# slowkow/scde

Hardware: NVIDIA B200
Metric: genes/sec scde.expression.difference (100 boot) (higher is better)
Workload: dtype f64 + s8 fixed point (2^-29, exact int32 sums)

## Files before the change

### scde_b200/csrc/api.cu

```cuda
#include "../../include/scde_b200.h"
#include "common.cuh"
#include "hostmath.h"

#include <cfloat>
#include <cmath>
#include <cstdarg>
#include <cstring>
#include <string>
#include <chrono>
#include <exception>
#include <map>
#include <memory>
#include <new>
#include <atomic>
#include <thread>
#include <vector>

namespace scde {

static thread_local std::string g_err;

void set_error(const char *fmt, ...) {
    char buf[1024];
    va_list ap;
// ... 54 lines not shown
            cudaEvent_t e;
            if (cudaEventCreate(&e) != cudaSuccess) return -1;
            pool.push_back(e);
        }
        return (int)used++;
    }
    int begin(cudaStream_t st) {
        int i = get();
        if (i >= 0) cudaEventRecord(pool[i], st);
        return i;
    }
    void end(int stage, int e0, cudaStream_t st, int n_launch) {
        int i = get();
        if (i >= 0 && e0 >= 0) {
            cudaEventRecord(pool[i], st);
            spans.push_back({stage, e0, i});
        }
        launches[stage] += n_launch;
    }
    void collect(scde_b200_stats *s) {
        for (int i = 0; i < SCDE_B200_T_COUNT; ++i) {
            s->ms[i] = 0;
            s->launches[i] = launches[i];
        }
        for (auto &sp : spans) {
            float ms = 0;
            if (cudaEventElapsedTime(&ms, pool[sp.e0], pool[sp.e1]) == cudaSuccess) s->ms[sp.stage] += ms;
        }
        int tot = 0;
        for (int i = 0; i < SCDE_B200_T_TOTAL; ++i) tot += launches[i];
        s->launches[SCDE_B200_T_TOTAL] = tot;
    }
};

}

using namespace scde;

namespace {
struct DiffWorkspace;
}

static scde_b200_options default_options() {
    scde_b200_options o;
    memset(&o, 0, sizeof(o));
    o.contract_kernel = 0;
    o.zero_base = 1;
    o.fused_fixed_point = 1;
    o.lp_rows_kernel = 0;
    o.count_chunks = 8;
    o.split_front = 1;
    o.uniform_chunks = 0;
    o.pipeline_front = 1;
    o.item_order = 1;
    o.hot_rank = -1;
    o.cold_evict_first = 1;
    o.twin_batch_joints = 1;
    o.prune_pieces = 1;
    return o;
}

struct scde_b200_ctx {
    int device = 0;
    cudaStream_t stream = nullptr;
    int n_sm = 148;
    scde_b200_options opt = default_options();
    std::vector<scde_b200_ctx *> children;
    DiffWorkspace *ws = nullptr;
    bool ws_busy = false;
    DBuf<unsigned long long> epi_dbg;
    cudaStream_t copy_stream = nullptr;
    std::vector<cudaEvent_t> copy_events;
    int32_t *h_draws = nullptr;
    size_t h_draws_cap = 0;
};

namespace {

inline int table_ld(int K) { return K <= KP_TILED ? KP_TILED : round_up(K, 8); }

struct LpTable {
    int n_cells = 0, n_genes = 0, K = 0, ld = 0, ld_ridx = 0;
    int64_t n_rows = 0;
    double sentinel = 0;
    DBuf<int32_t> row_off, row_x, row_mode, row_cell, row_snap, ridx, n_unique, err, zero_row, based;
    DBuf<double> table, mu, lcfp, lcfpr, theta, maxcfp, cfp, l1, l2, rowc, scfp;
    DBuf<int8_t> q;
    DBuf<uint32_t> qrange;
    DBuf<int8_t> qb;
    DBuf<uint32_t> dedup_bits;
    DBuf<unsigned long long> work_counter;
    bool want_q = false, has_q = false;
    bool want_bounds = false;
    bool has_bounds = false;
    bool f64_rows = true;
    bool want_modes = true;
    bool fast_theta = false;
    bool zero_base = false;
    bool zero_compact = false;
};

#define TRY(x)                          \
    do {                                \
        int _r = (x);                   \
        if (_r != SCDE_B200_OK) return _r; \
    } while (0)

#define CHECK_CTX(ctx)                                                  \
    do {                                                                \
        if (!(ctx)) {                                                   \
            set_error("null context");                                  \
            return SCDE_B200_EINVAL;                                    \
        }                                                               \
        SCDE_CUDA(cudaSetDevice((ctx)->device));                        \
    } while (0)

constexpr int PRUNE_MIN_CELLS = 2500;

struct TablePlan {
    bool fast = false;
    bool q_any = false;
    bool q_fused = false;
    CellPrep prep{};
    void *rowc = nullptr;
    int32_t *rmode = nullptr;
    int8_t *qf = nullptr;
    uint32_t *qr = nullptr;
    int8_t *qb = nullptr;
    bool bounds = false;
};

TablePlan plan_table(const scde_b200_ctx *ctx, const LpTable &t, int local_theta) {
    TablePlan pl;
    pl.fast = t.fast_theta && !local_theta && t.K <= KP_TILED;
    pl.q_any = t.want_q && t.zero_base && t.ld == KP_TILED && t.K <= Q_MAX_K;
    pl.q_fused = pl.q_any && pl.fast && ctx->opt.fused_fixed_point;
    pl.bounds = pl.q_any && (t.want_bounds || (ctx->opt.prune_pieces && t.n_cells >= PRUNE_MIN_CELLS));
    return pl;
}

int prepare_cells(scde_b200_ctx *ctx, LpTable &t, TablePlan &pl, const double *models_dev, int ld_models,
                  const double *mag_dev, int local_theta, int sqlogit) {
    cudaStream_t st = ctx->stream;
    const size_t cl = (size_t)t.n_cells * t.ld;
    SCDE_CUDA(t.mu.ensure(cl));
    SCDE_CUDA(t.lcfp.ensure(cl));
    SCDE_CUDA(t.lcfpr.ensure(cl));
    if (local_theta) SCDE_CUDA(t.theta.ensure(cl));
    SCDE_CUDA(t.maxcfp.ensure(t.n_cells));
    if (pl.fast) {
        SCDE_CUDA(t.cfp.ensure(cl));
        SCDE_CUDA(t.l1.ensure(cl));
        SCDE_CUDA(t.l2.ensure(cl));
        SCDE_CUDA(t.scfp.ensure((size_t)t.n_cells));
    }
    if (t.zero_base) {
        SCDE_CUDA(t.zero_row.ensure((size_t)t.n_cells));
        SCDE_CUDA(t.based.ensure((size_t)t.n_cells));
    }
    pl.prep = CellPrep{t.mu.p, t.lcfp.p, t.lcfpr.p, local_theta ? t.theta.p : nullptr, t.maxcfp.p, t.ld,
                       pl.fast ? t.cfp.p : nullptr, pl.fast ? t.l1.p : nullptr, pl.fast ? t.l2.p : nullptr,
                       pl.fast ? t.scfp.p : nullptr};
    SCDE_CUDA(launch_cell_prep(models_dev, ld_models, t.n_cells, mag_dev, t.K, local_theta, sqlogit, pl.prep, st));
    return SCDE_B200_OK;
}

int reserve_rows(LpTable &t, TablePlan &pl, size_t rows) {
    t.zero_compact = pl.q_fused && t.zero_base;
    SCDE_CUDA(t.table.ensure((t.zero_compact ? (size_t)t.n_cells : rows) * t.ld));
    SCDE_CUDA(t.row_mode.ensure(rows));
    SCDE_CUDA(t.row_cell.ensure(rows));
    if (pl.fast) {
        SCDE_CUDA(t.rowc.ensure(4 * rows));
        SCDE_CUDA(t.row_snap.ensure(rows));
    }
    if (pl.q_any) {
        SCDE_CUDA(t.q.ensure(rows * q_row_bytes(t.K)));
        SCDE_CUDA(t.qrange.ensure(rows));
        if (pl.bounds) SCDE_CUDA(t.qb.ensure(rows * Q_BW));
        SCDE_CUDA(t.work_counter.ensure(1));
    }
    pl.rowc = pl.fast ? (void *)t.rowc.p : nullptr;
    pl.rmode = t.want_modes ? t.row_mode.p : nullptr;
    pl.qf = pl.q_fused ? t.q.p : nullptr;
    pl.qr = pl.q_fused ? t.qrange.p : nullptr;
    pl.qb = pl.q_fused && pl.bounds ? t.qb.p : nullptr;
    t.has_bounds = pl.bounds;
    return SCDE_B200_OK;
}

int launch_table_rows(scde_b200_ctx *ctx, const LpTable &t, const TablePlan &pl, CellRange cr, const double *models_dev,
                      int ld_models, int local_theta, int *nl) {
    cudaStream_t st = ctx->stream;
    const int n = cr.c1 - cr.c0;
    SCDE_CUDA(launch_row_cell(t.row_off.p, cr, t.row_cell.p, st));
    ++*nl;
    if (pl.fast) {
        SCDE_CUDA(launch_row_consts(models_dev, ld_models, t.row_off.p, cr, t.row_cell.p, t.row_x.p, pl.rowc, t.row_snap.p,
                                    pl.prep, t.K, st));
        ++*nl;
    }
    if (t.zero_base) {
        SCDE_CUDA(launch_zero_rows(t.row_off.p + cr.c0, t.row_x.p, n, t.zero_row.p + cr.c0, cr.row_cap, st));
        SCDE_CUDA(launch_lp_rows(models_dev, ld_models, cr, t.row_off.p, t.row_cell.p, t.row_x.p, pl.prep, t.K, local_theta,
                                 t.sentinel, t.table.p, t.ld, pl.rmode, 1, t.zero_row.p, nullptr, pl.rowc, t.row_snap.p, 1, pl.qf, pl.qr,
                                 st, 0, nullptr, t.zero_compact, pl.qb));
        SCDE_CUDA(launch_based_flags(t.table.p, t.ld, t.K, t.sentinel, t.zero_row.p + cr.c0, n, t.based.p + cr.c0, st,
                                     t.zero_compact ? cr.c0 : -1));
        SCDE_CUDA(launch_lp_rows(models_dev, ld_models, cr, t.row_off.p, t.row_cell.p, t.row_x.p, pl.prep, t.K, local_theta,
                                 t.sentinel, t.table.p, t.ld, pl.rmode, 2, t.zero_row.p, t.based.p, pl.rowc, t.row_snap.p,
                                 pl.q_fused ? 0 : 1, pl.qf, pl.qr, st, ctx->opt.lp_rows_kernel == 1, t.work_counter.p,
                                 t.zero_compact, pl.qb));
        *nl += 4;
    } else {
        SCDE_CUDA(launch_lp_rows(models_dev, ld_models, cr, t.row_off.p, t.row_cell.p, t.row_x.p, pl.prep, t.K, local_theta,
                                 t.sentinel, t.table.p, t.ld, pl.rmode, 0, nullptr, nullptr, pl.rowc, t.row_snap.p, 1, nullptr, nullptr,
                                 st));
        ++*nl;
    }
    return SCDE_B200_OK;
}

int fill_table(scde_b200_ctx *ctx, LpTable &t, const double *models_dev, int ld_models, const double *mag_dev,
               int local_theta, int sqlogit, StageTimer *tm) {
    cudaStream_t st = ctx->stream;
    TablePlan pl = plan_table(ctx, t, local_theta);
    TRY(reserve_rows(t, pl, (size_t)t.n_rows));
    int e0 = tm ? tm->begin(st) : -1;
    int nl = 1;
    TRY(prepare_cells(ctx, t, pl, models_dev, ld_models, mag_dev, local_theta, sqlogit));
    TRY(launch_table_rows(ctx, t, pl, CellRange{0, t.n_cells, (int64_t)t.n_rows}, models_dev, ld_models, local_theta, &nl));
    t.has_q = pl.q_any;
    t.f64_rows = !(pl.q_fused && t.zero_base);
    if (pl.q_any && !pl.q_fused) {
        SCDE_CUDA(launch_quantize_rows(t.table.p, t.ld, t.K, t.n_rows, t.q.p, t.qrange.p, pl.bounds ? t.qb.p : nullptr, st));
        ++nl;
    }
    if (tm) tm->end(SCDE_B200_T_LPTABLE, e0, st, nl);
    return SCDE_B200_OK;
}

enum class Contraction { I8, Tiled, Generic };
struct ContractChoice {
    Contraction kernel;
    bool forced = false;
};

ContractChoice contraction_choice(const scde_b200_ctx *ctx) {
    switch (ctx->opt.contract_kernel) {
    case 1: return {Contraction::Generic};
    case 2: return {Contraction::Tiled};
    case 3: return {Contraction::I8, true};
    default: return {Contraction::I8};
    }
}

int index_from_counts(scde_b200_ctx *ctx, LpTable &t, const int32_t *counts_dev, int64_t ldc, int g0, int G, int C,
                      StageTimer *tm, int64_t known_cap = 0) {
    cudaStream_t st = ctx->stream;
    t.n_cells = C;
    t.n_genes = G;
    t.ld_ridx = C;
    SCDE_CUDA(t.n_unique.ensure(C));
    SCDE_CUDA(t.row_off.ensure((size_t)C + 1));
    SCDE_CUDA(t.err.ensure(1));
    SCDE_CUDA(t.ridx.ensure((size_t)G * C));
    int e0 = tm ? tm->begin(st) : -1;
    SCDE_CUDA(cudaMemsetAsync(t.err.p, 0, sizeof(int32_t), st));
    SCDE_CUDA(t.dedup_bits.ensure(dedup_scratch_words(C)));
    SCDE_CUDA(launch_dedup_count(counts_dev, ldc, g0, G, C, t.n_unique.p, t.err.p, t.dedup_bits.p, st));
    SCDE_CUDA(launch_exclusive_scan(t.n_unique.p, t.row_off.p, C, nullptr, st));
    int64_t cap = known_cap;
    if (known_cap <= 0) {
        int32_t total = 0, err = 0;
        SCDE_CUDA(cudaMemcpyAsync(&total, t.row_off.p + C, sizeof(int32_t), cudaMemcpyDeviceToHost, st));
        SCDE_CUDA(cudaMemcpyAsync(&err, t.err.p, sizeof(int32_t), cudaMemcpyDeviceToHost, st));
        SCDE_CUDA(cudaStreamSynchronize(st));
        if (err & 1) {
            set_error("negative count in the count matrix");
            return SCDE_B200_EINVAL;
        }
        if (err & 2) {
            set_error("a cell has >= 32768 distinct count values among the processed genes (hash capacity)");
            return SCDE_B200_ELIMIT;
        }
        cap = total;
    }
    t.n_rows = cap;
    SCDE_CUDA(t.row_x.ensure((size_t)cap));
    SCDE_CUDA(launch_dedup_emit(counts_dev, ldc, g0, G, C, t.row_off.p, t.row_x.p, t.ridx.p, t.ld_ridx, t.err.p, cap,
                                t.dedup_bits.p, st));
    if (tm) tm->end(SCDE_B200_T_DEDUP, e0, st, 5);
    return SCDE_B200_OK;
}

struct JointScratch {
    DBuf<double> W[2], Z[2], T[2];
    DBuf<double> zpart, spart;
    DBuf<int8_t> W8[2];
    DBuf<uint32_t> SR[2];
    DBuf<int32_t> lst_row, lst_cell, lst_len, order;
    DBuf<unsigned long long> total;
    DBuf<double> zb[2];
    DBuf<int32_t> S[2], items, n_live;
    DBuf<uint8_t> live;
};

struct DiffWorkspace {
    DBuf<int32_t> counts;
    LpTable table;
    JointScratch scr;
    DBuf<double> jp[4];
    DBuf<double> post, bpost, apost;
    DBuf<double> tbuf;
};

struct DrawSets {
    int n = 1;
    const int32_t *gene_set = nullptr;
};

struct Joint {
    const int32_t *boot_idx_dev;
    int D;
    double *jp_dev;
};

int contract_joint_i8(scde_b200_ctx *ctx, const LpTable &t, const GeneLists &lists, JointScratch &scr, int n_w_rows,
                      int n_boot, const DrawSets &sets, double scale, const Joint *joints, int n_joints, int ld_jp,
                      int hot_rank, int32_t *status, StageTimer *tm, bool prune, unsigned long long *prune_stats) {
    cudaStream_t st = ctx->stream;
    const int passes = (n_boot + WP_TILED - 1) / WP_TILED;
    ContractI8Args q{};
    q.qtable = t.q.p;
    q.ldq = q_row_bytes(t.K);
    q.row_range = t.qrange.p;
    q.lists = lists;
    q.n_w_rows = n_w_rows;
    q.n_boot = n_boot;
    q.gene_set = sets.gene_set;
    q.set_w8 = (int64_t)passes * n_w_rows * Q_WB;
    q.set_z = (int64_t)passes * WP_TILED * KP_TILED;
    q.scale = scale;
    q.sentinel = t.sentinel;
    q.K = t.K;
    q.ld_jp = ld_jp;
    q.err = status;
    q.dbg = nullptr;
    q.item_order = ctx->opt.item_order;
    q.hot_rank = hot_rank;
    q.cold_evict_first = ctx->opt.cold_evict_first;
    q.ring_stages = ctx->opt.ring_stages;
    if (ctx->opt.epilogue_timing) {
        SCDE_CUDA(ctx->epi_dbg.ensure(3));
        SCDE_CUDA(cudaMemsetAsync(ctx->epi_dbg.p, 0, 3 * sizeof(unsigned long long), st));
        q.dbg = ctx->epi_dbg.p;
    }
    const bool pass_pairs = n_joints == 1 && passes > 1 && ctx->opt.twin_batch_joints;
    const int n_sides = (n_joints > 1 || pass_pairs) ? 2 : 1;
    const int max_genes = contract_tiled_max_genes();
    const int mp = t.n_genes < max_genes ? t.n_genes : max_genes;
    for (int i = 0; i < n_sides; ++i) {
        SCDE_CUDA(scr.T[i].ensure(contract_tiled_scratch_doubles(t.n_genes)));
        SCDE_CUDA(scr.SR[i].ensure(contract_i8_range_words(mp)));
        if (prune) SCDE_CUDA(scr.S[i].ensure(prune_bound_ints(mp)));
    }
    SCDE_CUDA(scr.spart.ensure(softmax_i8_scratch_doubles(mp)));
    if (prune) {
        for (int j = 0; j < n_joints; ++j) SCDE_CUDA(scr.zb[j].ensure(prune_zb_doubles(sets.n, n_boot)));
        SCDE_CUDA(scr.live.ensure((size_t)mp));
        SCDE_CUDA(scr.items.ensure((size_t)mp * q_pieces(t.K)));
        SCDE_CUDA(scr.n_live.ensure(1));
        q.qbound = t.qb.p;
        q.items = scr.items.p;
        q.n_live = scr.n_live.p;
    }
    auto side = [&](int j, int ps, int i) {
        return I8Side{scr.W8[j].p + (size_t)ps * n_w_rows * Q_WB, scr.Z[j].p + (size_t)ps * WP_TILED * KP_TILED, scr.T[i].p,
                      scr.SR[i].p, scr.S[i].p, scr.zb[j].p, joints[j].jp_dev, ps};
    };
    struct Launch {
        I8Side s[2];
        int n;
    };
    std::vector<Launch> launches;
    for (int ps = 0; ps < passes; ++ps) {
        if (n_joints > 1)
            launches.push_back({{side(0, ps, 0), side(1, ps, 1)}, 2});
        else if (pass_pairs && ps + 1 < passes) {
            launches.push_back({{side(0, ps, 0), side(0, ps + 1, 1)}, 2});
            ++ps;
        } else
            launches.push_back({{side(0, ps, 0)}, 1});
    }
    if (prune) {
        const int e0 = tm ? tm->begin(st) : -1;
        for (int j = 0; j < n_joints; ++j) SCDE_CUDA(launch_z_bounds(q, scr.Z[j].p, sets.n, scr.zb[j].p, st));
        if (tm) tm->end(SCDE_B200_T_BOUND, e0, st, n_joints);
    }
    const uint8_t *live = prune ? scr.live.p : nullptr;
    for (int g0 = 0; g0 < t.n_genes; g0 += max_genes) {
        const int n_pos = (t.n_genes - g0) < max_genes ? (t.n_genes - g0) : max_genes;
        for (const Launch &l : launches) {
            int e0 = tm ? tm->begin(st) : -1;
            for (int i = 0; i < l.n; ++i) SCDE_CUDA(launch_sentinel_ranges(q, g0, n_pos, l.s[i], st));
            if (tm) tm->end(SCDE_B200_T_OTHER, e0, st, l.n);
            if (prune) {
                e0 = tm ? tm->begin(st) : -1;
                SCDE_CUDA(launch_bound_pass(q, g0, n_pos, l.s, l.n, ctx->n_sm, st));
                SCDE_CUDA(launch_prune_items(q, g0, n_pos, l.s, l.n, scr.live.p, scr.items.p, scr.n_live.p, prune_stats, st));
                if (tm) tm->end(SCDE_B200_T_BOUND, e0, st, 3);
            }
            e0 = tm ? tm->begin(st) : -1;
            SCDE_CUDA(launch_contract_i8_pass(q, g0, n_pos, l.s, l.n, ctx->n_sm, st));
            if (tm) tm->end(SCDE_B200_T_CONTRACT, e0, st, 1);
            e0 = tm ? tm->begin(st) : -1;
            for (int i = 0; i < l.n; ++i) SCDE_CUDA(launch_softmax_i8(q, g0, n_pos, l.s[i], scr.spart.p, ctx->n_sm, st, live));
            if (tm) tm->end(SCDE_B200_T_SOFTMAX, e0, st, 2 * l.n);
        }
    }
    if (q.dbg) {
        unsigned long long h[3];
        SCDE_CUDA(cudaMemcpyAsync(h, q.dbg, sizeof(h), cudaMemcpyDeviceToHost, st));
        SCDE_CUDA(cudaStreamSynchronize(st));
        fprintf(stderr, "[scde_b200] tcgen05 epilogue: %llu items, %.0f cycles from accumulators ready to tensor memory released, "
                "MMA thread waited %.0f cycles per item for the release\n", h[1], h[1] ? (double)h[0] / h[1] : 0.0,
                h[1] ? (double)h[2] / h[1] : 0.0);
    }
    return SCDE_B200_OK;
}

int contract_joint_fp64(scde_b200_ctx *ctx, Contraction kernel, const LpTable &t, const GeneLists &lists,
                        JointScratch &scr, const double *Z, int n_w_rows, int n_boot, const DrawSets &sets, double scale,
                        double *jp_dev, int ld_jp, StageTimer *tm) {
    cudaStream_t st = ctx->stream;
    if (!t.f64_rows) {
        set_error("internal: the table was built in fixed point only but the FP64 contraction kernel was selected");
        return SCDE_B200_EINVAL;
    }
    ContractArgs a;
    a.table = t.table.p;
    a.ld_table = t.ld;
    a.lists = lists;
    a.W = scr.W[0].p;
    a.n_w_rows = n_w_rows;
    a.n_boot = n_boot;
    a.Z = Z;
    const int passes = (n_boot + WP_TILED - 1) / WP_TILED;
    a.gene_set = sets.gene_set;
    a.set_w_rows = (int64_t)passes * n_w_rows;
    a.set_z = (int64_t)passes * WP_TILED * t.ld;
    a.scale = scale;
    a.n_genes = t.n_genes;
    a.K = t.K;
    a.jp = jp_dev;
    a.ld_jp = ld_jp;
    a.debug = ctx->opt.debug_contract;
    const bool tiled = kernel != Contraction::Generic && contract_tiled_supported(a);
    if (kernel == Contraction::Tiled && !tiled) {
        set_error("tiled contraction kernel forced but unsupported for K=%d", t.K);
        return SCDE_B200_EINVAL;
    }
    const int e0 = tm ? tm->begin(st) : -1;
    int nl = 0;
    if (tiled) {
        SCDE_CUDA(scr.T[0].ensure(contract_tiled_scratch_doubles(t.n_genes)));
        SCDE_CUDA(launch_contract_tiled(a, ctx->n_sm, scr.T[0].p, st, &nl));
    }
    else
        SCDE_CUDA(launch_contract_generic(a, st, &nl));
    if (tm) tm->end(SCDE_B200_T_CONTRACT, e0, st, nl);
    return SCDE_B200_OK;
}

int run_joint(scde_b200_ctx *ctx, ContractChoice k, const LpTable &t, const int32_t *cell_ids_dev, int n_list,
              const Joint *joints, int n_joints, int n_boot, const DrawSets &sets, double scale, int ld_jp,
              JointScratch &scr, int32_t *status, StageTimer *tm, bool count_entries) {
    cudaStream_t st = ctx->stream;
    const int n_w_rows = round_up(n_list + 1, 16);
    const int passes = (n_boot + WP_TILED - 1) / WP_TILED;
    const int ld_lst = round_up(n_list, 32);
    const bool zb = t.zero_base && t.ld <= KP_TILED;
    auto i8_for = [&](const Joint &jt) {
        return zb && t.has_q && k.kernel == Contraction::I8 && contract_i8_supported(t.K, t.ld, ld_lst, jt.D);
    };
    if (n_joints > 1 && !(i8_for(joints[0]) && i8_for(joints[1]) && ctx->opt.twin_batch_joints)) {
        for (int j = 0; j < n_joints; ++j)
            TRY(run_joint(ctx, k, t, cell_ids_dev, n_list, joints + j, 1, n_boot, sets, scale, ld_jp, scr, status, tm,
                          count_entries));
        return SCDE_B200_OK;
    }
    const bool i8 = i8_for(joints[0]);
    if (k.forced && !i8) {
        set_error("tcgen05 int8 contraction forced but unsupported here (K=%d, zero-base form %d)", t.K, (int)zb);
        return SCDE_B200_EINVAL;
    }
    const int S = sets.n;
    const size_t w_set = (size_t)passes * n_w_rows * WS_TILED, z_set = (size_t)passes * WP_TILED * t.ld;
    const size_t w8_set = (size_t)passes * n_w_rows * Q_WB;
    SCDE_CUDA(scr.lst_row.ensure((size_t)t.n_genes * ld_lst));
    SCDE_CUDA(scr.lst_cell.ensure((size_t)t.n_genes * ld_lst));
    SCDE_CUDA(scr.lst_len.ensure((size_t)t.n_genes));
    SCDE_CUDA(scr.order.ensure((size_t)t.n_genes));
    SCDE_CUDA(scr.total.ensure(5));
    if (zb) SCDE_CUDA(scr.zpart.ensure(base_sum_scratch_doubles(n_boot, t.ld)));
    for (int j = 0; j < n_joints; ++j) {
        SCDE_CUDA(scr.W[j].ensure(S * w_set));
        if (zb) SCDE_CUDA(scr.Z[j].ensure(S * z_set));
        if (i8) SCDE_CUDA(scr.W8[j].ensure(S * w8_set));
    }
    const int e0 = tm ? tm->begin(st) : -1;
    GeneLists lists{scr.lst_row.p, scr.lst_cell.p, scr.lst_len.p, scr.order.p, ld_lst};
    const int hot_rank = i8 ? ctx->opt.hot_rank : -1;
    SCDE_CUDA(launch_build_lists(t.ridx.p, t.ld_ridx, cell_ids_dev, n_list, t.n_genes, zb ? t.zero_row.p : nullptr,
                                 zb ? t.based.p : nullptr, 0, lists, count_entries ? scr.total.p : nullptr, st, hot_rank,
                                 n_joints));
    for (int j = 0; j < n_joints; ++j) {
        const Joint &jt = joints[j];
        const size_t draws_set = (size_t)n_boot * jt.D;
        for (int s = 0; s < S; ++s)
            SCDE_CUDA(launch_build_w(jt.boot_idx_dev + s * draws_set, n_boot, jt.D, n_list, scr.W[j].p + s * w_set, n_w_rows,
                                     st));
        SCDE_CUDA(cudaMemsetAsync(jt.jp_dev, 0, sizeof(double) * (size_t)t.n_genes * ld_jp, st));
        if (zb)
            for (int s = 0; s < S; ++s)
                SCDE_CUDA(launch_base_sum(t.table.p, t.ld, t.zero_row.p, t.based.p, cell_ids_dev, n_list,
                                          scr.W[j].p + s * w_set, n_w_rows, n_boot, scr.Z[j].p + s * z_set, scr.zpart.p, st,
                                          t.zero_compact));
        if (i8) SCDE_CUDA(launch_w_to_i8(scr.W[j].p, S * n_w_rows, n_boot, scr.W8[j].p, status, st));
    }
    if (tm) tm->end(SCDE_B200_T_OTHER, e0, st, n_joints * ((zb ? 5 : 3) + (S - 1) * (zb ? 4 : 2)) + (i8 ? 1 : 0));
    if (!i8)
        return contract_joint_fp64(ctx, k.kernel, t, lists, scr, zb ? scr.Z[0].p : nullptr, n_w_rows, n_boot, sets, scale,
                                   joints[0].jp_dev, ld_jp, tm);
    return contract_joint_i8(ctx, t, lists, scr, n_w_rows, n_boot, sets, scale, joints, n_joints, ld_jp, hot_rank, status, tm,
                             t.has_bounds && ctx->opt.prune_pieces && n_list >= PRUNE_MIN_CELLS,
                             count_entries ? scr.total.p + 1 : nullptr);
}

int read_status(const int32_t *words, int32_t *host, int n, bool *rerun) {
    SCDE_CUDA(cudaMemcpy(host, words, sizeof(int32_t) * n, cudaMemcpyDeviceToHost));
    int32_t any = 0;
    for (int i = 0; i < n; ++i) any |= host[i];
    if (any & 2) {
        set_error("tcgen05 contraction kernel aborted (pipeline watchdog); use scde_b200_set_contract_kernel(ctx, 2)");
        return SCDE_B200_ECUDA;
    }
    *rerun = (any & (1 | 4)) != 0;
    return SCDE_B200_OK;
}

bool theta_all_regular(const double *models, int ld, int n_cells) {
    for (int c = 0; c < n_cells; ++c) {
        const double th = models[(size_t)5 * ld + c];
        if (!(th > 0) || !std::isfinite(th)) return false;
    }
    return true;
}

std::vector<int32_t> gen_boot(int seed, int n, int n_boot) {
    std::vector<int32_t> v((size_t)n_boot * n);
    scde_b200_boot_indices(seed, n, n_boot, v.data());
    return v;
}

template <class T>
int upload(DBuf<T> &d, const T *h, size_t n, cudaStream_t st) {
    SCDE_CUDA(d.ensure(n));
    if (n) SCDE_CUDA(cudaMemcpyAsync(d.p, h, n * sizeof(T), cudaMemcpyHostToDevice, st));
    return SCDE_B200_OK;
}

int validate_index(const int32_t *v, size_t n, int lo, int hi, const char *what) {
    for (size_t i = 0; i < n; ++i)
        if (v[i] < lo || v[i] >= hi) {
            set_error("%s[%zu] = %d outside [%d, %d)", what, i, v[i], lo, hi);
            return SCDE_B200_EINVAL;
        }
    return SCDE_B200_OK;
}

std::vector<double> grid_magnitudes(const double *prior_x, int K) {
    std::vector<double> mag(K);
    for (int k = 0; k < K; ++k) {
        double m = std::pow(10.0, prior_x[k]) - 1;
        if (m < 0) m = 0;
        mag[k] = std::log(m);
    }
    return mag;
}

struct BatchPools {
    std::vector<int32_t> off, pool;
};

int batch_pools(const int32_t *batch, int C, int L, BatchPools &bp) {
    bp.off.assign(L + 1, 0);
    for (int c = 0; c < C; ++c) {
        if (batch[c] >= L) {
            set_error("batch[%d] = %d outside [0, %d) (negative = NA)", c, batch[c], L);
            return SCDE_B200_EINVAL;
        }
        if (batch[c] >= 0) bp.off[batch[c] + 1]++;
    }
    for (int l = 0; l < L; ++l) bp.off[l + 1] += bp.off[l];
    bp.pool.resize(bp.off[L] > 0 ? bp.off[L] : 1);
    std::vector<int32_t> pos(bp.off.begin(), bp.off.end() - 1);
    for (int c = 0; c < C; ++c)
        if (batch[c] >= 0) bp.pool[pos[batch[c]]++] = c;
    return SCDE_B200_OK;
}

int batch_composition(const int32_t *batch, int L, const int32_t *cells, size_t n, std::vector<int32_t> &comp) {
    comp.assign(L, 0);
    int D = 0;
    for (size_t i = 0; i < n; ++i)
        if (batch[cells[i]] >= 0) {
            comp[batch[cells[i]]]++;
            ++D;
        }
    return D;
}

std::vector<int32_t> zero_slice(const int32_t *zero_index, int n_zero, int g0, int G) {
    std::vector<int32_t> zi(n_zero == 1 ? 1 : G);
    for (size_t i = 0; i < zi.size(); ++i) zi[i] = zero_index[n_zero == 1 ? 0 : g0 + i];
    return zi;
}

struct ModelSet {
    DBuf<double> m;
    int C = 0, local_theta = 0, sqlogit = 0;
    bool fast_theta = false;
};

int upload_models(ModelSet &s, const double *models, int C, int local_theta, int sqlogit, cudaStream_t st) {
    s.C = C;
    s.local_theta = local_theta;
    s.sqlogit = sqlogit;
    s.fast_theta = !local_theta && theta_all_regular(models, C, C);
    return upload(s.m, models, (size_t)C * 12, st);
}

int fill_rows(scde_b200_ctx *ctx, LpTable &t, const ModelSet &ms, const double *mag_dev, StageTimer *tm) {
    t.fast_theta = ms.fast_theta;
    return fill_table(ctx, t, ms.m.p, ms.C, mag_dev, ms.local_theta, ms.sqlogit, tm);
}

void init_table(const scde_b200_ctx *ctx, ContractChoice k, LpTable &t, int K, int C, bool fast_theta) {
    t.K = K;
    t.ld = table_ld(K);
    t.sentinel = -DBL_MAX / C / 1.1;
    t.fast_theta = fast_theta;
    t.zero_base = t.ld <= KP_TILED && ctx->opt.zero_base;
    t.want_q = k.kernel == Contraction::I8;
    t.want_modes = false;
}

int workspace_busy(const scde_b200_ctx *ctx) {
    if (!ctx->ws_busy) return SCDE_B200_OK;
    set_error("another expression_difference job is alive on this context (free it first)");
    return SCDE_B200_EINVAL;
}

int acquire_workspace(scde_b200_ctx *ctx) {
    TRY(workspace_busy(ctx));
    if (!ctx->ws) ctx->ws = new DiffWorkspace();
    ctx->ws_busy = true;
    return SCDE_B200_OK;
}

struct RatioPasses {
    RatioArgs main;
    RatioArgs batch;
    RatioArgs adjusted;
};

RatioPasses ratio_passes(int G, int K, int ld, const double *prior_y, const int32_t *zi, const int32_t *zi_adj, int n_zero) {
    const int nout = 2 * K - 1;
    RatioPasses r{};
    r.main.ld = ld;
    r.main.n_genes = G;
    r.main.n = K;
    r.main.prior = prior_y;
    r.main.zero_index = zi;
    r.main.n_zero = n_zero == 1 ? 1 : G;
    r.main.ld_post = round_up(nout, 8);
    r.batch = r.main;
    r.batch.zero_index = nullptr;
    r.batch.n_zero = 1;
    r.adjusted.ld = r.main.ld_post;
    r.adjusted.n_genes = G;
    r.adjusted.n = nout;
    r.adjusted.prior = nullptr;
    r.adjusted.zero_index = zi_adj;
    r.adjusted.n_zero = r.main.n_zero;
    r.adjusted.ld_post = round_up(2 * nout - 1, 8);
    return r;
}

int launch_ratio_passes(const RatioPasses &r, bool has_batch, cudaStream_t st) {
    SCDE_CUDA(launch_ratio_summary(r.main, st));
    if (has_batch) {
        SCDE_CUDA(launch_ratio_summary(r.batch, st));
        SCDE_CUDA(launch_ratio_summary(r.adjusted, st));
    }
    return SCDE_B200_OK;
}

struct OutPlace {
    int64_t ld, row0;
};

int download_summary(cudaStream_t st, int G, const int32_t *idx, const double *z, int32_t *idx_dst, double *z_dst,
// ... 745 lines not shown
    SCDE_CUDA(d1.ensure((size_t)n_rows * ld));
    SCDE_CUDA(d2.ensure((size_t)n_rows * ld));
    SCDE_CUDA(cudaMemcpyAsync(d_in.p, m1, sizeof(double) * sz, cudaMemcpyHostToDevice, st));
    SCDE_CUDA(launch_transpose_in(d_in.p, n_rows, n, d1.p, ld, st));
    SCDE_CUDA(cudaMemcpyAsync(d_in.p, m2, sizeof(double) * sz, cudaMemcpyHostToDevice, st));
    SCDE_CUDA(launch_transpose_in(d_in.p, n_rows, n, d2.p, ld, st));
    SCDE_CUDA(d_raw.ensure((size_t)n_rows * ldo));
    RatioArgs a{};
    a.p1 = d1.p;
    a.p2 = d2.p;
    a.ld = ld;
    a.n_genes = n_rows;
    a.n = n;
    a.ld_post = ldo;
    a.raw = d_raw.p;
    SCDE_CUDA(launch_ratio_summary(a, st));
    SCDE_CUDA(d_out.ensure((size_t)n_rows * nout));
    SCDE_CUDA(launch_transpose_out(d_raw.p, ldo, n_rows, nout, d_out.p, st));
    SCDE_CUDA(cudaMemcpyAsync(out, d_out.p, sizeof(double) * (size_t)n_rows * nout, cudaMemcpyDeviceToHost, st));
    SCDE_CUDA(cudaStreamSynchronize(st));
    return SCDE_B200_OK;
}

int scde_b200_ratio_posterior_summary(scde_b200_ctx *ctx, const double *pmat1, const double *pmat2, int32_t n_genes,
                                      int32_t n, const double *prior_y, const int32_t *zero_index, int32_t n_zero,
                                      int32_t *idx, double *z, double *posterior) {
    CHECK_CTX(ctx);
    if (!pmat1 || !pmat2 || n_genes < 0 || n < 1 || !zero_index || (n_zero != 1 && n_zero != n_genes)) {
        set_error("ratio_posterior_summary: bad arguments");
        return SCDE_B200_EINVAL;
    }
    if (n_genes == 0) return SCDE_B200_OK;
    TRY(validate_index(zero_index, (size_t)n_zero, 1, 2 * n, "zero_index"));
    cudaStream_t st = ctx->stream;
    const int nout = 2 * n - 1, ld = round_up(n, 8), ldo = round_up(nout, 8);
    DBuf<double> d_in, d1, d2, d_prior, d_post, d_out, d_z;
    DBuf<int32_t> d_zi, d_idx;
    const size_t sz = (size_t)n_genes * n;
    SCDE_CUDA(d_in.ensure(sz));
    SCDE_CUDA(d1.ensure((size_t)n_genes * ld));
    SCDE_CUDA(d2.ensure((size_t)n_genes * ld));
    SCDE_CUDA(cudaMemcpyAsync(d_in.p, pmat1, sizeof(double) * sz, cudaMemcpyHostToDevice, st));
    SCDE_CUDA(launch_transpose_in(d_in.p, n_genes, n, d1.p, ld, st));
    SCDE_CUDA(cudaMemcpyAsync(d_in.p, pmat2, sizeof(double) * sz, cudaMemcpyHostToDevice, st));
    SCDE_CUDA(launch_transpose_in(d_in.p, n_genes, n, d2.p, ld, st));
    if (prior_y) TRY(upload(d_prior, prior_y, (size_t)n, st));
    TRY(upload(d_zi, zero_index, (size_t)n_zero, st));
    SCDE_CUDA(d_idx.ensure((size_t)3 * n_genes));
    SCDE_CUDA(d_z.ensure((size_t)n_genes));
    if (posterior) SCDE_CUDA(d_post.ensure((size_t)n_genes * ldo));
    RatioArgs a{};
    a.p1 = d1.p;
    a.p2 = d2.p;
    a.ld = ld;
    a.n_genes = n_genes;
    a.n = n;
    a.prior = prior_y ? d_prior.p : nullptr;
    a.zero_index = d_zi.p;
    a.n_zero = n_zero;
    a.idx = d_idx.p;
    a.z = d_z.p;
    a.post = posterior ? d_post.p : nullptr;
    a.ld_post = ldo;
    SCDE_CUDA(launch_ratio_summary(a, st));
    if (idx) SCDE_CUDA(cudaMemcpyAsync(idx, d_idx.p, sizeof(int32_t) * 3 * (size_t)n_genes, cudaMemcpyDeviceToHost, st));
    if (z) SCDE_CUDA(cudaMemcpyAsync(z, d_z.p, sizeof(double) * (size_t)n_genes, cudaMemcpyDeviceToHost, st));
    if (posterior) {
        SCDE_CUDA(d_out.ensure((size_t)n_genes * nout));
        SCDE_CUDA(launch_transpose_out(d_post.p, ldo, n_genes, nout, d_out.p, st));
        SCDE_CUDA(cudaMemcpyAsync(posterior, d_out.p, sizeof(double) * (size_t)n_genes * nout, cudaMemcpyDeviceToHost, st));
    }
    SCDE_CUDA(cudaStreamSynchronize(st));
    return SCDE_B200_OK;
}

int scde_b200_expression_magnitude(scde_b200_ctx *ctx, const int32_t *counts, int32_t n_genes, int32_t n_cells,
                                   const double *corr_b, const double *corr_a, double *out) {
    CHECK_CTX(ctx);
    if (!counts || !corr_b || !corr_a || !out || n_genes < 0 || n_cells < 0) {
        set_error("expression_magnitude: bad arguments");
        return SCDE_B200_EINVAL;
    }
    const size_t n = (size_t)n_genes * n_cells;
    if (n == 0) return SCDE_B200_OK;
    cudaStream_t st = ctx->stream;
    DBuf<int32_t> d_c;
    DBuf<double> d_b, d_a, d_o;
    TRY(upload(d_c, counts, n, st));
    TRY(upload(d_b, corr_b, (size_t)n_cells, st));
    TRY(upload(d_a, corr_a, (size_t)n_cells, st));
    SCDE_CUDA(d_o.ensure(n));
    SCDE_CUDA(launch_magnitude(d_c.p, (int64_t)n, n_genes, d_b.p, d_a.p, d_o.p, st));
    SCDE_CUDA(cudaMemcpyAsync(out, d_o.p, sizeof(double) * n, cudaMemcpyDeviceToHost, st));
    SCDE_CUDA(cudaStreamSynchronize(st));
    return SCDE_B200_OK;
}

int scde_b200_failure_probability(scde_b200_ctx *ctx, const double *models, int32_t n_cells, const int32_t *counts,
                                  const double *magnitudes, int32_t n_genes, int32_t square_logit_conc, double *out) {
    CHECK_CTX(ctx);
    if (!models || (!counts && !magnitudes) || !out || n_cells < 1 || n_genes < 0) {
        set_error("failure_probability: bad arguments (either magnitudes or counts should be provided)");
        return SCDE_B200_EINVAL;
    }
    const size_t n = (size_t)n_genes * n_cells;
    if (n == 0) return SCDE_B200_OK;
    cudaStream_t st = ctx->stream;
    DBuf<double> d_models, d_mag, d_out;
    DBuf<int32_t> d_counts;
    TRY(upload(d_models, models, (size_t)n_cells * 12, st));
    if (magnitudes)
        TRY(upload(d_mag, magnitudes, n, st));
    else
        TRY(upload(d_counts, counts, n, st));
    SCDE_CUDA(d_out.ensure(n));
    SCDE_CUDA(launch_failure_probability(magnitudes ? nullptr : d_counts.p, magnitudes ? d_mag.p : nullptr, (int64_t)n, n_genes,
                                         d_models.p, n_cells, square_logit_conc, d_out.p, st));
    SCDE_CUDA(cudaMemcpyAsync(out, d_out.p, sizeof(double) * n, cudaMemcpyDeviceToHost, st));
    SCDE_CUDA(cudaStreamSynchronize(st));
    return SCDE_B200_OK;
}

int scde_b200_expression_prior(scde_b200_ctx *ctx, const double *models, int32_t n_cells, const int32_t *counts,
                               int32_t n_genes, int32_t square_logit_conc, int32_t length_out, double pseudo_count, double bw,
                               double max_quantile, double max_value, double *x, double *y, double *lp, double *grid_weight) {
    CHECK_CTX(ctx);
    if (!models || !counts || !x || !y || n_cells < 1 || n_genes < 1 || length_out < 1 || !(bw > 0) ||
        !(max_quantile >= 0 && max_quantile <= 1)) {
        set_error("expression_prior: bad arguments");
        return SCDE_B200_EINVAL;
    }
    cudaStream_t st = ctx->stream;
    const int64_t n = (int64_t)n_genes * n_cells;
    DBuf<double> d_models, d_v, d_w, d_part;
    DBuf<int32_t> d_counts;
    DBuf<unsigned long long> d_scal, d_hist, d_bins;
    TRY(upload(d_models, models, (size_t)n_cells * 12, st));
    TRY(upload(d_counts, counts, (size_t)n, st));
    SCDE_CUDA(d_v.ensure((size_t)n));
    SCDE_CUDA(d_w.ensure((size_t)n));
    const int nb = prior_pass1_blocks(n);
    SCDE_CUDA(d_part.ensure((size_t)nb));
    SCDE_CUDA(d_scal.ensure(2));
    SCDE_CUDA(cudaMemsetAsync(d_scal.p, 0, 2 * sizeof(unsigned long long), st));
    SCDE_CUDA(launch_prior_pass1(d_counts.p, n, n_genes, d_models.p, n_cells, square_logit_conc, d_v.p, d_w.p, d_part.p, d_scal.p,
                                 d_scal.p + 1, st));
    std::vector<double> part((size_t)nb);
    unsigned long long scal[2] = {0, 0};
    SCDE_CUDA(cudaMemcpyAsync(part.data(), d_part.p, sizeof(double) * nb, cudaMemcpyDeviceToHost, st));
    SCDE_CUDA(cudaMemcpyAsync(scal, d_scal.p, sizeof(scal), cudaMemcpyDeviceToHost, st));
    SCDE_CUDA(cudaStreamSynchronize(st));
    long double wsum = 0;
    for (int i = 0; i < nb; ++i) wsum += part[i];
    const int64_t m = (int64_t)scal[1];
    if (std::isnan(max_value)) {
        if (m < 1) {
            set_error("expression_prior: no finite expression magnitude");
            return SCDE_B200_EINVAL;
        }
        if (max_quantile >= 1.0) {
            max_value = prior_key_to_double(scal[0]);
        } else {
            SCDE_CUDA(d_hist.ensure(256));
            auto kth = [&](int64_t rank, double *out) -> int {
                unsigned long long prefix = 0;
                for (int shift = 56; shift >= 0; shift -= 8) {
                    unsigned long long h[256];
                    SCDE_CUDA(cudaMemsetAsync(d_hist.p, 0, sizeof(h), st));
                    SCDE_CUDA(launch_select_hist(d_v.p, n, prefix, shift, d_hist.p, st));
                    SCDE_CUDA(cudaMemcpyAsync(h, d_hist.p, sizeof(h), cudaMemcpyDeviceToHost, st));
                    SCDE_CUDA(cudaStreamSynchronize(st));
                    int b = 0;
                    for (; b < 255 && rank >= (int64_t)h[b]; ++b) rank -= (int64_t)h[b];
                    prefix |= (unsigned long long)b << shift;
                }
                *out = prior_key_to_double(prefix);
                return SCDE_B200_OK;
            };
            const double index = 1 + (double)(m - 1) * max_quantile, fuzz = 4 * DBL_EPSILON;
            const double lo = std::floor(index + fuzz), hi = std::ceil(index - fuzz);
            double qlo = 0, qhi = 0;
            TRY(kth((int64_t)lo - 1, &qlo));
            double h = index - lo;
            if (std::fabs(h) < fuzz) h = 0;
            if (h != 0) {
                TRY(kth((int64_t)hi - 1, &qhi));
                max_value = (1 - h) * qlo + h * qhi;
            } else {
                max_value = qlo;
            }
        }
    }
    const int n_user = 2 * length_out + 1;
    int nbin = n_user > 512 ? n_user : 512;
    if (nbin > 512) {
        int p2 = 1;
        while (p2 < nbin) p2 <<= 1;
        nbin = p2;
    }
    if (nbin > 16384) {
        set_error("expression_prior: length_out %d too large (working grid of %d points)", length_out, nbin);
        return SCDE_B200_ELIMIT;
    }
    const double from = -1 * max_value, to = max_value, lo = from - 4 * bw, up = to + 4 * bw;
    SCDE_CUDA(d_bins.ensure((size_t)nbin));
    SCDE_CUDA(cudaMemsetAsync(d_bins.p, 0, sizeof(unsigned long long) * nbin, st));
    SCDE_CUDA(launch_prior_bins(d_v.p, d_w.p, n, 1.0 / (double)wsum, lo, (up - lo) / (nbin - 1), nbin, d_bins.p, st));
    std::vector<unsigned long long> hb((size_t)nbin);
    SCDE_CUDA(cudaMemcpyAsync(hb.data(), d_bins.p, sizeof(unsigned long long) * nbin, cudaMemcpyDeviceToHost, st));
    SCDE_CUDA(cudaStreamSynchronize(st));
    std::vector<double> yb((size_t)nbin), dx((size_t)n_user), dy((size_t)n_user);
    for (int i = 0; i < nbin; ++i) yb[i] = (double)(long long)hb[i] / 4611686018427387904.0;
    density_from_bins(yb.data(), nbin, lo, up, bw, n_user, from, to, dx.data(), dy.data());
    const int K = length_out + 1;
    long double ys = 0;
    for (int k = 0; k < K; ++k) {
        x[k] = dx[length_out + k];
        double v = dy[length_out + k];
        if (std::isnan(v)) v = 0;
        y[k] = v + pseudo_count / n_genes;
        ys += y[k];
    }
    for (int k = 0; k < K; ++k) {
        y[k] /= (double)ys;
        if (lp) lp[k] = std::log(y[k]);
    }
    if (grid_weight) {
        double prev = std::pow(10.0, x[0]) - 1;
        for (int k = 0; k < K; ++k) {
            const double edge = x[k] + (k < K - 1 ? (x[k + 1] - x[k]) / 2 : 0);
            const double cur = std::pow(10.0, edge) - 1;
            grid_weight[k] = cur - prev;
            prev = cur;
        }
    }
    return SCDE_B200_OK;
}

int scde_b200_probe_contract_i8(scde_b200_ctx *ctx, const int8_t *qtable, int32_t n_rows, int32_t n_grid,
                                const uint32_t *row_range, const int8_t *w8, int32_t n_w_rows, const int32_t *lst_row,
                                const int32_t *lst_cell, const int32_t *lst_len, int32_t n_genes, int32_t ld_lst,
                                double *t_out, int32_t *flags_out) {
    return scde_b200_probe_prune_i8(ctx, qtable, n_rows, n_grid, row_range, nullptr, nullptr, w8, n_w_rows, lst_row, lst_cell,
                                    lst_len, n_genes, ld_lst, t_out, nullptr, nullptr, nullptr, nullptr, flags_out);
}

int scde_b200_probe_prune_i8(scde_b200_ctx *ctx, const int8_t *qtable, int32_t n_rows, int32_t n_grid,
                             const uint32_t *row_range, const int8_t *qbound, const double *z, const int8_t *w8,
                             int32_t n_w_rows, const int32_t *lst_row, const int32_t *lst_cell, const int32_t *lst_len,
                             int32_t n_genes, int32_t ld_lst, double *t_out, double *lb_out, double *ub_out,
                             uint8_t *live_out, double *exp_out, int32_t *flags_out) {
    CHECK_CTX(ctx);
    if (qbound && (!lb_out || !ub_out || !live_out)) {
        set_error("probe_prune_i8: bad arguments");
        return SCDE_B200_EINVAL;
    }
    if (!qtable || !w8 || !lst_row || !lst_cell || !lst_len || !t_out || n_rows < 1 || n_genes < 1 || n_w_rows < 1 ||
        !contract_i8_supported(n_grid, KP_TILED, ld_lst, 1) || n_genes > contract_tiled_max_genes()) {
        set_error("probe_contract_i8: bad arguments");
        return SCDE_B200_EINVAL;
    }
    for (int g = 0; g < n_genes; ++g) {
        if (lst_len[g] < 0 || lst_len[g] > ld_lst) {
            set_error("probe_contract_i8: lst_len[%d] out of range", g);
            return SCDE_B200_EINVAL;
        }
    }
    TRY(validate_index(lst_row, (size_t)n_genes * ld_lst, 0, n_rows, "lst_row"));
    TRY(validate_index(lst_cell, (size_t)n_genes * ld_lst, 0, n_w_rows, "lst_cell"));
    cudaStream_t st = ctx->stream;
    DBuf<int8_t> d_q, d_w;
    DBuf<int32_t> d_row, d_cell, d_len, status;
    DBuf<uint32_t> d_rr, d_sr;
    DBuf<double> d_t;
    const int ldq = q_row_bytes(n_grid);
    TRY(upload(d_q, qtable, (size_t)n_rows * ldq, st));
    if (row_range) TRY(upload(d_rr, row_range, (size_t)n_rows, st));
    TRY(upload(d_w, w8, (size_t)n_w_rows * Q_WB, st));
    TRY(upload(d_row, lst_row, (size_t)n_genes * ld_lst, st));
    TRY(upload(d_cell, lst_cell, (size_t)n_genes * ld_lst, st));
    TRY(upload(d_len, lst_len, (size_t)n_genes, st));
    const size_t nt = (size_t)n_genes * WP_TILED * KP_TILED;
    SCDE_CUDA(d_t.ensure(nt));
    SCDE_CUDA(d_sr.ensure(contract_i8_range_words(n_genes)));
    SCDE_CUDA(cudaMemsetAsync(d_t.p, 0, sizeof(double) * nt, st));
    SCDE_CUDA(status.ensure(1));
    SCDE_CUDA(cudaMemsetAsync(status.p, 0, sizeof(int32_t), st));
    ContractI8Args q{};
    q.qtable = d_q.p;
    q.ldq = ldq;
    q.row_range = row_range ? d_rr.p : nullptr;
    q.lists = GeneLists{d_row.p, d_cell.p, d_len.p, nullptr, ld_lst};
    q.n_w_rows = n_w_rows;
    q.n_boot = WP_TILED;
    q.scale = 1.0;
    q.sentinel = -1.0e300;
    q.K = n_grid;
    q.ld_jp = 0;
    q.err = status.p;
    q.item_order = ctx->opt.item_order;
    q.hot_rank = -1;
    q.cold_evict_first = 0;
    q.ring_stages = ctx->opt.ring_stages;
    I8Side side{d_w.p, nullptr, d_t.p, d_sr.p, nullptr, nullptr, nullptr, 0};
    SCDE_CUDA(launch_sentinel_ranges(q, 0, n_genes, side, st));
    DBuf<int8_t> d_qb;
    DBuf<double> d_z, d_zb, d_lb, d_ub;
    DBuf<int32_t> d_s, d_items, d_nlive;
    DBuf<uint8_t> d_live;
    if (qbound) {
        TRY(upload(d_qb, qbound, (size_t)n_rows * Q_BW, st));
        if (z) TRY(upload(d_z, z, (size_t)WP_TILED * KP_TILED, st));
        q.qbound = d_qb.p;
        SCDE_CUDA(d_zb.ensure(prune_zb_doubles(1, WP_TILED)));
        SCDE_CUDA(d_s.ensure(prune_bound_ints(n_genes)));
        SCDE_CUDA(d_lb.ensure((size_t)n_genes * WP_TILED));
        SCDE_CUDA(d_ub.ensure((size_t)n_genes * WP_TILED * 4));
        SCDE_CUDA(d_live.ensure((size_t)n_genes));
        SCDE_CUDA(d_items.ensure((size_t)n_genes * q_pieces(n_grid)));
        SCDE_CUDA(d_nlive.ensure(1));
        side.S = d_s.p;
        side.zb = d_zb.p;
        SCDE_CUDA(launch_z_bounds(q, z ? d_z.p : nullptr, 1, d_zb.p, st));
        SCDE_CUDA(launch_bound_pass(q, 0, n_genes, &side, 1, ctx->n_sm, st));
        SCDE_CUDA(launch_prune_items(q, 0, n_genes, &side, 1, d_live.p, d_items.p, d_nlive.p, nullptr, st, d_lb.p, d_ub.p));
    }
    SCDE_CUDA(launch_contract_i8_pass(q, 0, n_genes, &side, 1, ctx->n_sm, st));
    SCDE_CUDA(launch_finalize_t(q, n_genes, side, st));
    SCDE_CUDA(cudaMemcpyAsync(t_out, d_t.p, sizeof(double) * nt, cudaMemcpyDeviceToHost, st));
    if (qbound) {
        SCDE_CUDA(cudaMemcpyAsync(lb_out, d_lb.p, sizeof(double) * n_genes * WP_TILED, cudaMemcpyDeviceToHost, st));
        SCDE_CUDA(cudaMemcpyAsync(ub_out, d_ub.p, sizeof(double) * n_genes * WP_TILED * 4, cudaMemcpyDeviceToHost, st));
        SCDE_CUDA(cudaMemcpyAsync(live_out, d_live.p, n_genes, cudaMemcpyDeviceToHost, st));
    }
    if (exp_out) SCDE_CUDA(launch_exp_probe(exp_out, st));
    SCDE_CUDA(cudaStreamSynchronize(st));
    int32_t f = 0;
    bool rerun = false;
    const int r = read_status(status.p, &f, 1, &rerun);
    if (flags_out) *flags_out = f;
    return r;
}

}

struct scde_b200_diff_job {
    int G = 0, C = 0, K = 0, n_boot = 0, n_levels = 0;
    int want_post = 0, has_batch = 0;
    int n_group[2] = {0, 0};
    int n_zero = 1;
    DiffWorkspace *ws = nullptr;
    scde_b200_ctx *owner = nullptr;
    ModelSet models;
    ModelSet bmodels;
    DBuf<double> mag, prior_y;
    DBuf<int32_t> cell_ids[2];
    DBuf<int32_t> boot[4];
    int D[4] = {0, 0, 0, 0};
    DrawChunks chunks;
    DBuf<int32_t> gene_set;
    DBuf<int32_t> zi, zi_adj;
    DBuf<int32_t> idx, bidx, aidx;
    DBuf<double> z, bz, az;
    DBuf<int32_t> status;
    StageTimer timer;
    bool ran = false;
    int64_t known_rows = 0;
    bool rows_unchecked = false;
    int copy_chunks = 0;
    std::vector<int> copy_bounds;
    int split_chunks = 0;
    int64_t front_cap = 0;
    TablePlan front_plan;
    const int32_t *boot_ptr[4] = {nullptr, nullptr, nullptr, nullptr};
    std::vector<int32_t> ids[2];
    std::unique_ptr<int32_t[]> gen[4];
    const scde_b200_diff_args *deferred_args = nullptr;
};

int upload_draws(scde_b200_ctx *ctx, scde_b200_diff_job *j, const scde_b200_diff_args *a, bool pinned = false) {
    cudaStream_t st = ctx->stream;
    const int C = j->C;
    const int S = j->chunks.n_sets();
    const int n_joints = j->has_batch ? 4 : 2;
    BatchPools bp;
    std::vector<int32_t> comp[2];
    for (int i = 0; i < 2; ++i) j->D[i] = j->n_group[i];
    if (j->has_batch) {
        TRY(batch_pools(a->batch, C, a->n_batch_levels, bp));
        for (int i = 0; i < 2; ++i)
            j->D[2 + i] = batch_composition(a->batch, a->n_batch_levels, j->ids[i].data(), j->ids[i].size(), comp[i]);
    }
    for (int i = 0; i < n_joints; ++i)
        if (a->boot_idx[i] && j->D[i] > 0)
            TRY(validate_index(a->boot_idx[i], (size_t)a->n_boot * j->D[i], 0, i < 2 ? j->D[i] : C,
                               i < 2 ? "boot_idx" : "batch boot_idx"));
    int32_t *dst[4] = {nullptr, nullptr, nullptr, nullptr};
    int32_t *dev = nullptr;
    if (pinned) {
        size_t total = 0;
        for (int i = 0; i < n_joints; ++i) total += (size_t)S * a->n_boot * j->D[i];
        if (total > ctx->h_draws_cap) {
            if (ctx->h_draws) cudaFreeHost(ctx->h_draws);
            ctx->h_draws = nullptr;
            ctx->h_draws_cap = 0;
            SCDE_CUDA(cudaHostAlloc((void **)&ctx->h_draws, sizeof(int32_t) * total, cudaHostAllocMapped));
            ctx->h_draws_cap = total;
        }
        SCDE_CUDA(cudaHostGetDevicePointer((void **)&dev, ctx->h_draws, 0));
        size_t off = 0;
        for (int i = 0; i < n_joints; ++i) {
            dst[i] = ctx->h_draws + off;
            j->boot_ptr[i] = dev + off;
            off += (size_t)S * a->n_boot * j->D[i];
        }
    } else {
        for (int i = 0; i < n_joints; ++i)
            if (!a->boot_idx[i]) {
                j->gen[i].reset(new int32_t[(size_t)S * a->n_boot * j->D[i]]);
                dst[i] = j->gen[i].get();
            }
    }
    std::vector<std::pair<int, int>> tasks;
    for (int i = 0; i < n_joints; ++i) {
        if (a->boot_idx[i]) {
            if (pinned) tasks.emplace_back(i, -1);
            continue;
        }
        for (int s = 0; s < S; ++s) tasks.emplace_back(i, s);
    }
    const std::vector<int32_t> &seeds = j->chunks.seeds;
    TRY(parallel_for((int)tasks.size(), [&](int t) -> int {
        const int i = tasks[t].first, s = tasks[t].second;
        const size_t per = (size_t)a->n_boot * j->D[i];
        if (s < 0) {
            memcpy(dst[i], a->boot_idx[i], sizeof(int32_t) * per);
            return SCDE_B200_OK;
        }
        int32_t *out = dst[i] + s * per;
        if (i < 2) return scde_b200_boot_indices(seeds[s], j->n_group[i], a->n_boot, out);
        return scde_b200_batch_boot_indices(seeds[s], a->n_batch_levels, bp.off.data(), bp.pool.data(), comp[i - 2].data(),
                                            a->n_boot, out);
    }));
    if (pinned) return SCDE_B200_OK;
    for (int i = 0; i < n_joints; ++i) {
        TRY(upload(j->boot[i], a->boot_idx[i] ? a->boot_idx[i] : dst[i], (size_t)S * a->n_boot * j->D[i], st));
        j->boot_ptr[i] = j->boot[i].p;
    }
    SCDE_CUDA(cudaStreamSynchronize(st));
    return SCDE_B200_OK;
}

constexpr int N_COUNT_CHUNKS_DEFAULT = 8;
static int n_count_chunks(const scde_b200_ctx *ctx) {
    const int n = ctx->opt.count_chunks > 0 ? ctx->opt.count_chunks : N_COUNT_CHUNKS_DEFAULT;
    return n < 1 ? 1 : (n > 64 ? 64 : n);
}

int start_count_copies(scde_b200_ctx *ctx, scde_b200_diff_job *j, const int32_t *counts_host, int64_t ld_host) {
    const int G = j->G, C = j->C;
    const int N_COUNT_CHUNKS = n_count_chunks(ctx);
    if (!ctx->copy_stream) SCDE_CUDA(cudaStreamCreateWithFlags(&ctx->copy_stream, cudaStreamNonBlocking));
    while ((int)ctx->copy_events.size() < N_COUNT_CHUNKS + 1) {
        cudaEvent_t e;
        SCDE_CUDA(cudaEventCreateWithFlags(&e, cudaEventDisableTiming));
        ctx->copy_events.push_back(e);
    }
    SCDE_CUDA(cudaEventRecord(ctx->copy_events[N_COUNT_CHUNKS], ctx->stream));
    SCDE_CUDA(cudaStreamWaitEvent(ctx->copy_stream, ctx->copy_events[N_COUNT_CHUNKS], 0));
    std::vector<int> &bounds = j->copy_bounds;
    bounds.assign(1, 0);
    j->split_chunks = 0;
    auto add_equal = [&](int lo, int hi, int n) {
        n = n < 1 ? 1 : n;
        const int step = round_up((hi - lo + n - 1) / n, 32);
        for (int c = lo + step; c < hi; c += step) bounds.push_back(c);
        bounds.push_back(hi);
    };
    int split = 0;
    if (!j->ids[0].empty() && ctx->opt.split_front) {
        int last0 = 0;
        for (int c : j->ids[0]) last0 = c > last0 ? c : last0;
        split = round_up(last0 + 1, 32);
    }
    if (N_COUNT_CHUNKS >= 4 && C >= 64 * N_COUNT_CHUNKS && !ctx->opt.uniform_chunks) {
        const int first = round_up(C / 20, 32), last = round_up(C / 16, 32);
        if (split >= 2 * first && split <= C - 2 * last && split <= (C / 4) * 3) {
            int nA = (int)((double)N_COUNT_CHUNKS * split / C + 0.5);
            nA = nA < 2 ? 2 : (nA > N_COUNT_CHUNKS - 2 ? N_COUNT_CHUNKS - 2 : nA);
            bounds.push_back(first);
            add_equal(first, split, nA - 1);
            j->split_chunks = (int)bounds.size() - 1;
            add_equal(split, C - last - ((C - last) % 32), N_COUNT_CHUNKS - nA - 1);
            bounds.push_back(C);
        } else {
            const int mid = round_up((C - first - last + N_COUNT_CHUNKS - 3) / (N_COUNT_CHUNKS - 2), 32);
            bounds.push_back(first);
            for (int i = 0; i < N_COUNT_CHUNKS - 2 && bounds.back() + mid < C - last; ++i) bounds.push_back(bounds.back() + mid);
            if (bounds.back() < C - last) bounds.push_back(C - last - ((C - last) % 32));
            if (bounds.back() <= bounds[bounds.size() - 2]) bounds.pop_back();
            bounds.push_back(C);
        }
    } else {
        const int chunk = round_up((C + N_COUNT_CHUNKS - 1) / N_COUNT_CHUNKS, 32);
        for (int c0 = chunk; c0 < C; c0 += chunk) bounds.push_back(c0);
        bounds.push_back(C);
    }
    while ((int)ctx->copy_events.size() < (int)bounds.size() + 1) {
        cudaEvent_t e;
        SCDE_CUDA(cudaEventCreateWithFlags(&e, cudaEventDisableTiming));
        ctx->copy_events.push_back(e);
    }
    j->copy_chunks = 0;
    for (int n_ch = 0; n_ch + 1 < (int)bounds.size(); ++n_ch) {
        const int c0 = bounds[n_ch], n = bounds[n_ch + 1] - c0;
        j->copy_chunks = n_ch + 1;
        SCDE_CUDA(cudaMemcpy2DAsync(j->ws->counts.p + (size_t)c0 * G, sizeof(int32_t) * G, counts_host + (size_t)c0 * ld_host,
                                    sizeof(int32_t) * (size_t)ld_host, sizeof(int32_t) * G, n, cudaMemcpyHostToDevice,
                                    ctx->copy_stream));
        SCDE_CUDA(cudaEventRecord(ctx->copy_events[n_ch], ctx->copy_stream));
    }
    return SCDE_B200_OK;
}

static int gene_range(const scde_b200_diff_args *a, int *g0, int *g1) {
    *g0 = a->gene_begin;
    *g1 = a->gene_end;
    if (*g0 == 0 && *g1 == 0) *g1 = a->n_genes;
    if (*g0 < 0 || *g1 > a->n_genes || *g0 >= *g1) {
        set_error("gene range [%d, %d) invalid for %d genes", *g0, *g1, a->n_genes);
        return SCDE_B200_EINVAL;
    }
    return SCDE_B200_OK;
}

static int diff_upload_impl(scde_b200_ctx *ctx, ContractChoice k, const scde_b200_diff_args *a, int32_t want_posteriors,
                            scde_b200_diff_job **out, bool defer_counts) {
    if (!a || !out) return SCDE_B200_EINVAL;
    *out = nullptr;
    if (!a->counts || !a->models || !a->prior_x || !a->prior_y || !a->group || a->n_genes < 1 || a->n_cells < 1 ||
        a->n_grid < 2 || a->n_boot < 1) {
        set_error("expression_difference: bad arguments");
        return SCDE_B200_EINVAL;
    }
    int g0 = 0, g1 = 0;
    TRY(gene_range(a, &g0, &g1));
    TRY(check_draw_chunks(a->draw_chunks, a->boot_idx[0] || a->boot_idx[1] || a->boot_idx[2] || a->boot_idx[3],
                          "expression_difference"));
    const int G = g1 - g0, C = a->n_cells, K = a->n_grid;
    std::vector<int32_t> ids[2];
    for (int c = 0; c < C; ++c)
        if (a->group[c] == 0 || a->group[c] == 1) ids[a->group[c]].push_back(c);
    if (ids[0].empty() || ids[1].empty()) {
        set_error("both groups need at least one cell");
        return SCDE_B200_EINVAL;
    }
    const bool has_batch = a->batch != nullptr && a->n_batch_levels > 1;
    if (a->n_zero != 1 && a->n_zero != a->n_genes) {
        set_error("n_zero must be 1 or n_genes");
        return SCDE_B200_EINVAL;
    }
    if (!a->zero_index || (has_batch && !a->zero_index_adjusted)) {
        set_error("zero_index (and zero_index_adjusted with batch) are required");
        return SCDE_B200_EINVAL;
    }
    cudaStream_t st = ctx->stream;
    TRY(acquire_workspace(ctx));
    scde_b200_diff_job *j = new scde_b200_diff_job();
    j->ws = ctx->ws;
    j->owner = ctx;
    auto fail = [&](int r) {
        if (j->copy_chunks) cudaStreamSynchronize(ctx->copy_stream);
        ctx->ws_busy = false;
        delete j;
        return r;
    };
#define JTRY(x)                                \
    do {                                       \
        int _r = (x);                          \
        if (_r != SCDE_B200_OK) return fail(_r); \
    } while (0)
#define JCUDA(x)                                                                    \
    do {                                                                            \
        cudaError_t _e = (x);                                                       \
        if (_e != cudaSuccess) return fail(cuda_fail(_e, #x, __FILE__, __LINE__));   \
    } while (0)
    j->G = G;
    j->C = C;
    j->K = K;
    j->n_boot = a->n_boot;
    j->want_post = want_posteriors;
    j->has_batch = has_batch;
    j->n_levels = has_batch ? a->n_batch_levels : 0;
    j->n_zero = a->n_zero;
    const bool trace = ctx->opt.trace != 0;
    const auto tu0 = std::chrono::steady_clock::now();
    JCUDA(j->ws->counts.ensure((size_t)G * C));
    const auto tu1 = std::chrono::steady_clock::now();
    if (!defer_counts)
        JCUDA(cudaMemcpy2DAsync(j->ws->counts.p, sizeof(int32_t) * G, a->counts + g0, sizeof(int32_t) * (size_t)a->n_genes,
                                sizeof(int32_t) * G, C, cudaMemcpyHostToDevice, st));
    if (trace && !defer_counts) {
        JCUDA(cudaStreamSynchronize(st));
        const auto tu2 = std::chrono::steady_clock::now();
        fprintf(stderr, "[scde_b200] upload: counts buffer %.2f ms, counts H2D (%.1f MB) %.2f ms\n",
                std::chrono::duration<double, std::milli>(tu1 - tu0).count(), sizeof(int32_t) * (double)G * C / 1e6,
                std::chrono::duration<double, std::milli>(tu2 - tu1).count());
    }
    JTRY(upload_models(j->models, a->models, C, a->local_theta, a->square_logit_conc, st));
    if (has_batch && a->batch_models && a->batch_models != a->models)
        JTRY(upload_models(j->bmodels, a->batch_models, C, a->batch_local_theta, a->batch_square_logit_conc, st));
    JTRY(upload(j->prior_y, a->prior_y, (size_t)K, st));
    const std::vector<double> mag = grid_magnitudes(a->prior_x, K);
    JTRY(upload(j->mag, mag.data(), (size_t)K, st));
    for (int i = 0; i < 2; ++i) {
        j->n_group[i] = (int)ids[i].size();
        JTRY(upload(j->cell_ids[i], ids[i].data(), ids[i].size(), st));
    }
    j->ids[0] = ids[0];
    j->ids[1] = ids[1];
    j->chunks = draw_chunks_of(a->n_genes, a->draw_chunks, a->seed, g0, g1);
    if (j->chunks.n_sets() > 1) JTRY(upload(j->gene_set, j->chunks.gene_set.data(), j->chunks.gene_set.size(), st));
    if (defer_counts)
        j->deferred_args = a;
    else
        JTRY(upload_draws(ctx, j, a));
    {
        const std::vector<int32_t> zi = zero_slice(a->zero_index, a->n_zero, g0, G);
// ... 913 lines not shown
```

### scde_b200/csrc/common.cuh

```cuda
#pragma once
#include <cuda_runtime.h>
#include <cstdint>
#include <cstdio>

namespace scde {

constexpr int KP_TILED = 416;
constexpr int WP_TILED = 104;
constexpr int WS_TILED = 108;

inline int round_up(int x, int m) { return (x + m - 1) / m * m; }

void set_error(const char *fmt, ...);
int cuda_fail(cudaError_t e, const char *what, const char *file, int line);

#define SCDE_CUDA(expr)                                                                   \
    do {                                                                                  \
        cudaError_t _e = (expr);                                                          \
        if (_e != cudaSuccess) return ::scde::cuda_fail(_e, #expr, __FILE__, __LINE__);   \
    } while (0)

struct CellPrep {
    double *mu, *lcfp, *lcfpr, *theta;
    double *maxcfp;
    int ld;
    double *cfp, *l1, *l2;
    double *scfp;
};
cudaError_t launch_cell_prep(const double *models, int ld_models, int n_cells, const double *mag, int K,
                             int local_theta, int sqlogit, CellPrep prep, cudaStream_t st);
struct CellRange {
    int c0, c1;
    int64_t row_cap;
};
cudaError_t launch_row_cell(const int32_t *row_off, CellRange cr, int32_t *row_cell, cudaStream_t st);
cudaError_t launch_zero_rows(const int32_t *row_off, const int32_t *row_x, int n_cells, int32_t *zero_row, int64_t row_cap,
                             cudaStream_t st);
cudaError_t launch_based_flags(const double *table, int ld_table, int K, double sentinel, const int32_t *zero_row,
                               int n_cells, int32_t *based, cudaStream_t st, int zero_compact_c0 = -1);
cudaError_t launch_lp_rows(const double *models, int ld_models, CellRange cr, const int32_t *row_off,
                           const int32_t *row_cell_map, const int32_t *row_x, CellPrep prep, int K,
                           int local_theta, double sentinel, double *table, int ld_table, int32_t *row_mode, int which,
                           const int32_t *zero_row, const int32_t *based, void *row_const, const int32_t *row_snap,
                           int write_f64, int8_t *qtable, uint32_t *row_range, cudaStream_t st, int legacy_q_rows = 0,
                           unsigned long long *work_counter = nullptr, int zero_compact = 0, int8_t *qbound = nullptr);
cudaError_t launch_row_consts(const double *models, int ld_models, const int32_t *row_off, CellRange cr,
                              const int32_t *row_cell, const int32_t *row_x, void *row_const, int32_t *row_snap,
                              CellPrep prep, int K, cudaStream_t st);

size_t dedup_scratch_words(int n_cells);
cudaError_t launch_dedup_count(const int32_t *counts, int64_t ld_counts, int g0, int G, int n_cells,
                               int32_t *n_unique, int32_t *err_flag, uint32_t *scratch, cudaStream_t st);
cudaError_t launch_exclusive_scan(const int32_t *in, int32_t *out, int n, const int32_t *base_dev, cudaStream_t st);
cudaError_t launch_dedup_emit(const int32_t *counts, int64_t ld_counts, int g0, int G, int n_cells,
                              const int32_t *row_off, int32_t *row_x, int32_t *ridx, int ld_ridx,
                              int32_t *err_flag, int64_t row_cap , const uint32_t *scratch,
                              cudaStream_t st);
cudaError_t launch_uci_to_ridx(const int32_t *uci, int G, int n_cells, const int32_t *ucl_off, int32_t *ridx,
                               int ld_ridx, cudaStream_t st);

cudaError_t launch_build_w(const int32_t *boot_idx, int n_boot, int D, int n_list, double *W, int n_w_rows,
                           cudaStream_t st);
struct GeneLists {
    int32_t *row, *cell, *len, *order;
    int ld;
};
cudaError_t launch_build_lists(const int32_t *ridx, int ld_ridx, const int32_t *cell_ids, int n_list, int n_genes,
                               const int32_t *zero_row, const int32_t *based, int pad_row, GeneLists out,
                               unsigned long long *total_entries ,
                               cudaStream_t st, int hot_rank = -1, int count_times = 1);
size_t base_sum_scratch_doubles(int n_boot, int ld_table);
cudaError_t launch_base_sum(const double *table, int ld_table, const int32_t *zero_row, const int32_t *based,
                            const int32_t *cell_ids, int n_list, const double *W, int n_w_rows, int n_boot, double *Z,
                            double *scratch, cudaStream_t st, int zero_compact = 0);
struct ContractArgs {
    const double *table;
    int ld_table;
    GeneLists lists;
    const double *W;
    int n_w_rows;
    int n_boot;
    const double *Z;
    const int32_t *gene_set;
    int64_t set_w_rows, set_z;
    double scale;
    int n_genes, K;
    double *jp;
    int ld_jp;
    int debug = 0;
};
cudaError_t launch_contract_generic(const ContractArgs &a, cudaStream_t st, int *n_launches);
size_t contract_tiled_scratch_doubles(int n_genes);
cudaError_t launch_contract_tiled(const ContractArgs &a, int n_sm, double *t_scratch, cudaStream_t st, int *n_launches);
bool contract_tiled_supported(const ContractArgs &a);
cudaError_t launch_ensemble(const double *table, int ld_table, const int32_t *ridx, int ld_ridx, int n_cells, int n_genes,
                            int K, double *jp, int ld_jp, double *rownorm_scratch, int64_t n_rows, cudaStream_t st);
cudaError_t launch_gather_modes(const int32_t *ridx, int ld_ridx, int G, int n_cells, const int32_t *row_mode,
                                const double *mag, double *modes, cudaStream_t st);
cudaError_t launch_gather_post(const int32_t *ridx, int ld_ridx, int G, int n_cells, const double *table,
                               int ld_table, int K, double sentinel, double minlogprob, double *post,
                               cudaStream_t st);
cudaError_t launch_transpose_out(const double *src, int ld_src, int G, int K, double *dst, cudaStream_t st);
cudaError_t launch_transpose_in(const double *src, int G, int K, double *dst, int ld_dst, cudaStream_t st);
cudaError_t launch_fp64_peak(double *sink, int iters, int blocks, cudaStream_t st);
cudaError_t launch_softmax_avg(double *T, const int32_t *order, int K, int n_boot_pass, double scale, double *jp,
                               int ld_jp, int accumulate, int n_pos, cudaStream_t st);
int contract_tiled_max_genes();

constexpr int Q_NV = 5;
constexpr int Q_FRAC = 29;
constexpr int Q_PW = 102;
constexpr int Q_PIECE = 512;
constexpr int Q_MAX_K = 4 * Q_PW;
constexpr int Q_WB = 128;
constexpr uint32_t Q_RANGE_IRREGULAR = 0xFFFFFFFFu;
inline int q_pieces(int K) { return (K + Q_PW - 1) / Q_PW; }
constexpr int Q_BW = 128;
constexpr int Q_BSLOTS = Q_BW / 2;
constexpr int Q_UB_PTS = 16, Q_UB_N = KP_TILED / Q_UB_PTS;
constexpr int Q_LB_STEP = 12, Q_LB_OFF = 6, Q_LB_N = 35;
static_assert(Q_UB_N + Q_LB_N <= Q_BSLOTS && Q_LB_STEP * (Q_LB_N - 1) + Q_LB_OFF < KP_TILED, "bound row layout");
__host__ __device__ inline void q_bound_store(int8_t *brow, int slot, int v) {
    const int lo = (int)(int8_t)(v & 0xFF);
    brow[slot] = (int8_t)lo;
    brow[Q_BSLOTS + slot] = (int8_t)((v - lo) >> 8);
}
inline int q_row_bytes(int K) { return q_pieces(K) * Q_PIECE; }
#ifdef __CUDACC__
__device__ inline long long q_value_at(const int8_t *q, int k) {
    const int pc = k / Q_PW, i = k - pc * Q_PW;
    long long x = 0;
#pragma unroll
    for (int pl = Q_NV - 1; pl >= 0; --pl) x = x * 256 + q[pc * Q_PIECE + pl * Q_PW + i];
    return x;
}
__device__ inline void q_bound_row(const int8_t *q, int K, uint32_t range, int8_t *brow, int l, int LW) {
    int klo = 0, khi = K - 1;
    if (range != Q_RANGE_IRREGULAR) {
        klo = (int)(range & 0xFFFFu);
        khi = (int)(range >> 16);
    }
    for (int u = l; u < Q_UB_N; u += LW) {
        long long m = INT64_MIN;
        for (int k = max(u * Q_UB_PTS, klo); k < (u + 1) * Q_UB_PTS && k <= khi; ++k) m = max(m, q_value_at(q, k));
        q_bound_store(brow, u, m == INT64_MIN ? 0 : (int)((m + ((1ll << 24) - 1)) >> 24));
    }
    for (int c = l; c < Q_LB_N; c += LW) {
        const int k = Q_LB_STEP * c + Q_LB_OFF;
        q_bound_store(brow, Q_UB_N + c, k < K ? (int)(q_value_at(q, k) >> 24) : 0);
    }
}
#endif
cudaError_t launch_quantize_rows(const double *table, int ld_table, int K, int64_t n_rows, int8_t *qtable,
                                 uint32_t *row_range, int8_t *qbound, cudaStream_t st);
cudaError_t launch_w_to_i8(const double *W, int n_w_rows, int n_boot, int8_t *W8, int32_t *flag, cudaStream_t st);
struct ContractI8Args {
    const int8_t *qtable;
    int ldq;
    const uint32_t *row_range;
    GeneLists lists;
    int n_w_rows;
    int n_boot;
    const int32_t *gene_set;
    int64_t set_w8, set_z;
    double scale;
    double sentinel;
    int K;
    int ld_jp;
    int32_t *err;
    unsigned long long *dbg;
    int item_order;
    int hot_rank;
    int cold_evict_first;
    int ring_stages;
    const int8_t *qbound;
    const int32_t *items;
    const int32_t *n_live;
};
struct I8Side {
    const int8_t *W8;
    const double *Z;
    double *T;
    uint32_t *SR;
    int32_t *S;
    const double *zb;
    double *jp;
    int pass;
};
constexpr int32_t LIST_HOT_BIT = 1 << 30;
bool contract_i8_supported(int K, int ld_table, int ld_lst, int n_draws);
size_t contract_i8_range_words(int n_genes);
cudaError_t launch_sentinel_ranges(const ContractI8Args &a, int g0, int n_pos, const I8Side &s, cudaStream_t st);
cudaError_t launch_contract_i8_pass(const ContractI8Args &a, int g0, int n_pos, const I8Side *s, int n_sides, int n_sm,
                                    cudaStream_t st);
size_t softmax_i8_scratch_doubles(int n_pos);
cudaError_t launch_softmax_i8(const ContractI8Args &a, int g0, int n_pos, const I8Side &s, double *part_scratch, int n_sm,
                              cudaStream_t st, const uint8_t *live = nullptr);
size_t prune_zb_doubles(int n_sets, int n_boot);
cudaError_t launch_z_bounds(const ContractI8Args &a, const double *Z, int n_sets, double *zb, cudaStream_t st);
size_t prune_bound_ints(int n_pos);
cudaError_t launch_bound_pass(const ContractI8Args &a, int g0, int n_pos, const I8Side *s, int n_sides, int n_sm,
                              cudaStream_t st);
cudaError_t launch_prune_items(const ContractI8Args &a, int g0, int n_pos, const I8Side *s, int n_sides, uint8_t *live,
                               int32_t *items, int32_t *n_live, unsigned long long *stats, cudaStream_t st,
                               double *lb_out = nullptr, double *ub_out = nullptr);
cudaError_t launch_exp_probe(double *out_host, cudaStream_t st);
cudaError_t launch_finalize_t(const ContractI8Args &a, int n_pos, const I8Side &s, cudaStream_t st);

struct RatioContrast {
    const double *p1, *p2;
    int32_t *idx;
    double *z;
    double *post;
};
struct RatioArgs {
    const double *p1, *p2;
    int ld;
    int n_genes, n;
    const double *prior;
    const int32_t *zero_index;
    int n_zero;
    int32_t *idx;
    double *z;
    double *post;
    int ld_post;
    double *raw;
    const RatioContrast *contrasts;
    int n_contrasts;
};
cudaError_t launch_ratio_summary(const RatioArgs &a, cudaStream_t st);
cudaError_t launch_magnitude(const int32_t *counts, int64_t n, int G, const double *corr_b, const double *corr_a,
                             double *out, cudaStream_t st);


int prior_pass1_blocks(int64_t n);
cudaError_t launch_failure_probability(const int32_t *counts, const double *mag, int64_t n, int G, const double *models, int C,
                                       int sq, double *out, cudaStream_t st);
cudaError_t launch_prior_pass1(const int32_t *counts, int64_t n, int G, const double *models, int C, int sq, double *v, double *w,
                               double *part , unsigned long long *vmax_key,
                               unsigned long long *n_finite, cudaStream_t st);
cudaError_t launch_select_hist(const double *v, int64_t n, unsigned long long prefix, int shift, unsigned long long *hist,
                               cudaStream_t st);
cudaError_t launch_prior_bins(const double *v, const double *w, int64_t n, double inv_sum, double lo, double xdelta, int nbin,
                              unsigned long long *bins, cudaStream_t st);
double prior_key_to_double(unsigned long long k);

}
```

### scde_b200/csrc/contract_i8.cu

```cuda
#include "common.cuh"
#include "ptx_sm100.cuh"
#include "fastmath.cuh"
#include <cfloat>
#include <cmath>
#include <cstdlib>

namespace scde {
namespace {

using namespace ptx;

constexpr int Q_ES = 32;
constexpr int Q_NS = 10;
constexpr int Q_A_BYTES = Q_ES * Q_WB;
constexpr int Q_B_BYTES = Q_ES * Q_PIECE;
constexpr int Q_STAGE_BYTES = Q_A_BYTES + Q_B_BYTES;
constexpr int Q_EPILOGUE_WARPS = 8;
constexpr int q_threads(int pg) { return (4 * pg + Q_EPILOGUE_WARPS + 1) * 32; }
constexpr int Q_EPI_ROUNDS = (Q_PW + 7) / 8;
constexpr int Q_TMEM_COLS = 512;
constexpr long long Q_WATCHDOG_CYCLES = 4000000000ll;
static_assert(Q_NV * Q_PW <= Q_TMEM_COLS && Q_NV * Q_PW <= Q_PIECE, "a piece is one pass of tensor memory");
static_assert((Q_PW & 1) == 0, "the epilogue reads pairs of columns");

struct I8Smem {
    uint64_t full[Q_NS];
    uint64_t empty[Q_NS];
    uint64_t acc_full, acc_empty;
    uint32_t tmem_base;
    volatile int abort;
};
constexpr int Q_XBUF_BYTES = Q_EPILOGUE_WARPS * 2048;
constexpr size_t q_smem_bytes(int ns) { return 1024  + (size_t)ns * Q_STAGE_BYTES + Q_XBUF_BYTES + sizeof(I8Smem); }

struct I8Params {
    const int8_t *qtable;
    int64_t ldq;
    const int32_t *lst_row, *lst_cell, *lst_len, *order;
    int64_t ld_lst;
    const int8_t *W8;
    const int32_t *gene_set;
    int64_t set_w8;
    long long *T;
    int n_boot;
    int n_pos;
    int n_pieces;
    int32_t *err;
    unsigned long long *dbg;
    const int8_t *W8b;
    long long *Tb;
    int twin;
    int piece_major;
    int cold_evict_first;
    const int32_t *items;
    const int32_t *n_live;
};

__device__ __forceinline__ bool wait_or_abort(I8Smem &sm, uint64_t *bar, uint32_t parity) {
    if (mbar_try_wait(bar, parity)) return true;
    const long long t0 = clock64();
    while (!mbar_try_wait(bar, parity)) {
        if (sm.abort) return false;
        if (clock64() - t0 > Q_WATCHDOG_CYCLES) {
            sm.abort = 1;
            return false;
        }
    }
    return true;
}

struct Item {
    int pos, piece;
};
__device__ __forceinline__ int item_code(const I8Params &p, int item) {
    item >>= p.twin;
    return p.items ? __ldg(p.items + item) : item;
}
__device__ __forceinline__ Item decode_item(const I8Params &p, int item) {
    Item it;
    item = item_code(p, item);
    if (p.piece_major) {
        it.piece = item / p.n_pos;
        it.pos = item - it.piece * p.n_pos;
    } else {
        it.pos = item / p.n_pieces;
        it.piece = item - it.pos * p.n_pieces;
    }
    return it;
}
__device__ __forceinline__ int64_t item_gene(const I8Params &p, int item) {
    item = item_code(p, item);
    const int pos = p.piece_major ? item % p.n_pos : item / p.n_pieces;
    return p.order ? p.order[pos] : pos;
}

template <int DOFF, int SOFF>
__device__ __forceinline__ void cp_async16_at(uint32_t dst_smem, const void *src) {
    asm volatile("cp.async.cg.shared.global [%0+%2], [%1+%3], 16;" ::"r"(dst_smem), "l"(src), "n"(DOFF), "n"(SOFF) : "memory");
}
template <int DOFF, int SOFF>
__device__ __forceinline__ void cp_async16_hint_at(uint32_t dst_smem, const void *src, uint64_t policy) {
    asm volatile("cp.async.cg.shared.global.L2::cache_hint [%0+%2], [%1+%3], 16, %4;" ::"r"(dst_smem), "l"(src), "n"(DOFF), "n"(SOFF),
                 "l"(policy)
                 : "memory");
}
template <int Q_PGROUPS, bool HINT, int NS, bool BOUND>
__device__ __forceinline__ void run_producer(const I8Params &p, I8Smem &sm, uint32_t stage0, int n_items, int warp, int lane) {
    uint64_t pol_hot = 0, pol_cold = 0;
    if (HINT) {
        asm volatile("createpolicy.fractional.L2::evict_last.b64 %0, 1.0;" : "=l"(pol_hot));
        if (p.cold_evict_first)
            asm volatile("createpolicy.fractional.L2::evict_first.b64 %0, 1.0;" : "=l"(pol_cold));
        else
            asm volatile("createpolicy.fractional.L2::evict_normal.b64 %0, 1.0;" : "=l"(pol_cold));
    }
    const int grp = warp >> 2, kg = warp & 3;
    const int l7 = lane & 7, l3 = lane >> 3;
    const uint32_t d0 = (uint32_t)kg * 1024u + (uint32_t)l3 * 128u + (uint32_t)((l7 ^ l3) << 4);
    const uint32_t d1 = (uint32_t)kg * 1024u + (uint32_t)(l3 + 4) * 128u + (uint32_t)((l7 ^ (l3 + 4)) << 4);
    int slot_b = 0;
    uint32_t fill_b = 0;
    int item = blockIdx.x;
    int64_t gene_n = 0, wset_n = 0;
    int len_n = 0;
    if (item < n_items) {
        gene_n = item_gene(p, item);
        len_n = p.lst_len[gene_n];
        if (p.gene_set) wset_n = p.gene_set[gene_n] * p.set_w8;
    }
    for (; item < n_items; item += gridDim.x) {
        const Item it = decode_item(p, item);
        const int64_t gene = gene_n, wset = wset_n;
        const int nst = (len_n + Q_ES - 1) / Q_ES;
        if (item + (int)gridDim.x < n_items) {
            gene_n = item_gene(p, item + gridDim.x);
            len_n = p.lst_len[gene_n];
            if (p.gene_set) wset_n = p.gene_set[gene_n] * p.set_w8;
        }
        const int8_t *qbase = p.qtable + (BOUND ? 0 : (int64_t)it.piece * Q_PIECE) + l7 * 16;
        const int8_t *wbase = ((p.twin && (item & 1)) ? p.W8b : p.W8) + l7 * 16 + wset;
        const int32_t *lrow = p.lst_row + gene * p.ld_lst + kg * 8 + l3;
        const int32_t *lcell = p.lst_cell + gene * p.ld_lst + kg * 8 + l3;
        int32_t r0a = 0, r1a = 0, c0a = 0, c1a = 0, r0b = 0, r1b = 0, c0b = 0, c1b = 0;
        auto load_block = [&](int t, int32_t &r0, int32_t &r1, int32_t &c0, int32_t &c1) {
            const int s = grp + Q_PGROUPS * (8 * t + l7);
            r0 = r1 = c0 = c1 = 0;
            if (s < nst) {
                r0 = __ldg(lrow + s * Q_ES);
                r1 = __ldg(lrow + s * Q_ES + 4);
                c0 = __ldg(lcell + s * Q_ES);
                c1 = __ldg(lcell + s * Q_ES + 4);
            }
        };
        load_block(0, r0a, r1a, c0a, c1a);
        load_block(1, r0b, r1b, c0b, c1b);
        int slot = slot_b + grp;
        uint32_t fill = fill_b;
        if (slot >= NS) {
            slot -= NS;
            ++fill;
        }
        for (int t = 0; grp + Q_PGROUPS * 8 * t < nst; ++t) {
#pragma unroll
            for (int u = 0; u < 8; ++u) {
                const int s = grp + Q_PGROUPS * (8 * t + u);
                if (s < nst) {
                    const int from = (lane & 24) | u;
                    const int32_t row0 = __shfl_sync(0xffffffffu, r0a, from), row1 = __shfl_sync(0xffffffffu, r1a, from);
                    const int32_t cel0 = __shfl_sync(0xffffffffu, c0a, from), cel1 = __shfl_sync(0xffffffffu, c1a, from);
                    const uint32_t sA = stage0 + (uint32_t)slot * Q_STAGE_BYTES;
                    const uint32_t sB0 = sA + Q_A_BYTES + d0, sB1 = sA + Q_A_BYTES + d1;
                    const int8_t *src0 = qbase + (int64_t)row0 * p.ldq;
                    const int8_t *src1 = qbase + (int64_t)row1 * p.ldq;
                    const int8_t *w0 = wbase + (int64_t)(cel0 & ~LIST_HOT_BIT) * Q_WB;
                    const int8_t *w1 = wbase + (int64_t)(cel1 & ~LIST_HOT_BIT) * Q_WB;
                    if (fill > 0 && !wait_or_abort(sm, &sm.empty[slot], (fill - 1) & 1u)) return;
                    if (BOUND) {
                        cp_async16_at<0, 0>(sB0, src0);
                        cp_async16_at<0, 0>(sB1, src1);
                        cp_async16_at<0, 0>(sA + d0, w0);
                        cp_async16_at<0, 0>(sA + d1, w1);
                    } else if (HINT) {
                        const uint64_t pol0 = (cel0 & LIST_HOT_BIT) ? pol_hot : pol_cold;
                        const uint64_t pol1 = (cel1 & LIST_HOT_BIT) ? pol_hot : pol_cold;
                        cp_async16_hint_at<0, 0>(sB0, src0, pol0);
                        cp_async16_hint_at<0, 0>(sB1, src1, pol1);
                        cp_async16_hint_at<4096, 128>(sB0, src0, pol0);
                        cp_async16_hint_at<4096, 128>(sB1, src1, pol1);
                        cp_async16_hint_at<8192, 256>(sB0, src0, pol0);
                        cp_async16_hint_at<8192, 256>(sB1, src1, pol1);
                        cp_async16_hint_at<12288, 384>(sB0, src0, pol0);
                        cp_async16_hint_at<12288, 384>(sB1, src1, pol1);
                        cp_async16_hint_at<0, 0>(sA + d0, w0, pol_hot);
                        cp_async16_hint_at<0, 0>(sA + d1, w1, pol_hot);
                    } else {
                        cp_async16_at<0, 0>(sB0, src0);
                        cp_async16_at<0, 0>(sB1, src1);
                        cp_async16_at<4096, 128>(sB0, src0);
                        cp_async16_at<4096, 128>(sB1, src1);
                        cp_async16_at<8192, 256>(sB0, src0);
                        cp_async16_at<8192, 256>(sB1, src1);
                        cp_async16_at<12288, 384>(sB0, src0);
                        cp_async16_at<12288, 384>(sB1, src1);
                        cp_async16_at<0, 0>(sA + d0, w0);
                        cp_async16_at<0, 0>(sA + d1, w1);
                    }
                    cp_async_mbar_arrive_noinc(&sm.full[slot]);
                    slot += Q_PGROUPS;
                    if (slot >= NS) {
                        slot -= NS;
                        ++fill;
                    }
                }
            }
            r0a = r0b;
            r1a = r1b;
            c0a = c0b;
            c1a = c1b;
            load_block(t + 2, r0b, r1b, c0b, c1b);
        }
        slot_b += nst % NS;
        fill_b += (uint32_t)(nst / NS);
        if (slot_b >= NS) {
            slot_b -= NS;
            ++fill_b;
        }
    }
}

template <int NS, bool BOUND>
__device__ __forceinline__ void run_mma(const I8Params &p, I8Smem &sm, uint32_t stage0, uint32_t tmem, int n_items) {
    const uint32_t idesc = umma_idesc_s8_mn(128, BOUND ? Q_BW : 256);
    int slot = 0;
    uint32_t fill = 0, n_done = 0;
    int item = blockIdx.x;
    int len_n = item < n_items ? p.lst_len[item_gene(p, item)] : 0;
    for (; item < n_items; item += gridDim.x, ++n_done) {
        const int nst = (len_n + Q_ES - 1) / Q_ES;
        if (item + (int)gridDim.x < n_items) len_n = p.lst_len[item_gene(p, item + gridDim.x)];
        if (n_done > 0) {
            const long long t0 = p.dbg ? clock64() : 0;
            if (!wait_or_abort(sm, &sm.acc_empty, (n_done - 1) & 1u)) return;
            tc_fence_after_sync();
            if (p.dbg) atomicAdd(p.dbg + 2, (unsigned long long)(clock64() - t0));
        }
        for (int s = 0; s < nst; ++s) {
            if (!wait_or_abort(sm, &sm.full[slot], fill & 1u)) return;
            fence_proxy_async_smem();
            tc_fence_after_sync();
            const uint32_t sA = stage0 + (uint32_t)slot * Q_STAGE_BYTES;
            const uint32_t sB = sA + Q_A_BYTES;
            const uint64_t da = umma_desc_sw128(sA, 4096u, 1024u);
            umma_s8(tmem, da, umma_desc_sw128(sB, 4096u, 1024u), idesc, s > 0);
            if (!BOUND) umma_s8(tmem + 256u, da, umma_desc_sw128(sB + 2u * 4096u, 4096u, 1024u), idesc, s > 0);
            umma_commit(&sm.empty[slot]);
            if (++slot == NS) {
                slot = 0;
                ++fill;
            }
        }
        if (nst > 0)
            umma_commit(&sm.acc_full);
        else
            mbar_arrive(&sm.acc_full);
    }
}

__device__ __forceinline__ void run_epilogue(const I8Params &p, I8Smem &sm, uint32_t xbuf, uint32_t tmem, int n_items, int ewarp,
                                             int lane) {
    const int qd = ewarp & 3, half = ewarp >> 2;
    const uint32_t tlane = tmem + ((uint32_t)(qd * 32) << 16);
    const uint32_t xw = xbuf + (uint32_t)ewarp * 2048u;
    const int rb = lane >> 2, rc = lane & 3;
    const int r_begin = half ? (Q_EPI_ROUNDS + 1) / 2 : 0, r_end = half ? Q_EPI_ROUNDS : (Q_EPI_ROUNDS + 1) / 2;
    uint32_t n_done = 0;
    for (int item = blockIdx.x; item < n_items; item += gridDim.x, ++n_done) {
        const Item it = decode_item(p, item);
        const int64_t gene = p.order ? p.order[it.pos] : it.pos;
        const bool empty_list = p.lst_len[gene] <= 0;
        while (!mbar_try_wait(&sm.acc_full, n_done & 1u)) {
            __nanosleep(200);
            if (sm.abort) return;
        }
        tc_fence_after_sync();
        const long long t_ready = p.dbg ? clock64() : 0;
        long long *Tbase = ((p.twin && (item & 1)) ? p.Tb : p.T) + ((int64_t)it.pos * WP_TILED + qd * 32) * KP_TILED + it.piece * Q_PW;
        for (int rd = r_begin; rd < r_end; ++rd) {
            const int i0 = rd * 8;
            const int n = Q_PW - i0 < 8 ? Q_PW - i0 : 8;
            uint32_t r[Q_NV][8];
#pragma unroll
            for (int pl = 0; pl < Q_NV; ++pl)
#pragma unroll
                for (int j = 0; j < 8; ++j) r[pl][j] = 0u;
            if (!empty_list) {
#pragma unroll
                for (int pl = 0; pl < Q_NV; ++pl) tmem_ld_32x32b_x8(tlane + (uint32_t)(pl * Q_PW + i0), r[pl]);
                tmem_wait_ld();
            }
            long long out[8];
#pragma unroll
            for (int j = 0; j < 8; ++j) {
                const int32_t a = (int32_t)r[0][j] + ((int32_t)r[1][j] << 8);
                const int32_t c = (int32_t)r[2][j] + ((int32_t)r[3][j] << 8);
                out[j] = (long long)a + ((long long)c << 16) + ((long long)(int32_t)r[4][j] << 32);
            }
#pragma unroll
            for (int j = 0; j < 4; ++j)
                asm volatile("st.shared.v2.b64 [%0], {%1, %2};" ::"r"(xw + 512u * j + (uint32_t)(((lane + 8 * j) & 31) << 4)),
                             "l"(out[2 * j]), "l"(out[2 * j + 1])
                             : "memory");
            __syncwarp();
#pragma unroll
            for (int i = 0; i < 4; ++i) {
                const int bw = rb + 8 * i;
                long long v0, v1;
                asm volatile("ld.shared.v2.b64 {%0, %1}, [%2];" : "=l"(v0), "=l"(v1)
                             : "r"(xw + 512u * rc + (uint32_t)(((bw + 8 * rc) & 31) << 4)) : "memory");
                if (qd * 32 + bw < p.n_boot && 2 * rc < n)
                    __stcs(reinterpret_cast<longlong2 *>(Tbase + (int64_t)bw * KP_TILED + i0 + 2 * rc), make_longlong2(v0, v1));
            }
            __syncwarp();
        }
        tc_fence_before_sync();
        mbar_arrive(&sm.acc_empty);
        if (p.dbg && ewarp == 0 && lane == 0) {
            atomicAdd(p.dbg, (unsigned long long)(clock64() - t_ready));
            atomicAdd(p.dbg + 1, 1ull);
        }
    }
}

__device__ __forceinline__ void run_bound_epilogue(const I8Params &p, I8Smem &sm, uint32_t tmem, int n_items, int ewarp, int lane) {
    const int qd = ewarp & 3, half = ewarp >> 2;
    const uint32_t tcol = tmem + ((uint32_t)(qd * 32) << 16) + (uint32_t)(half * 64);
    const int boot = qd * 32 + lane;
    uint32_t n_done = 0;
    for (int item = blockIdx.x; item < n_items; item += gridDim.x, ++n_done) {
        const int pos = item >> p.twin;
        const bool empty_list = p.lst_len[p.order ? p.order[pos] : pos] <= 0;
        while (!mbar_try_wait(&sm.acc_full, n_done & 1u)) {
            __nanosleep(200);
            if (sm.abort) return;
        }
        tc_fence_after_sync();
        int4 *dst = reinterpret_cast<int4 *>(reinterpret_cast<int32_t *>((p.twin && (item & 1)) ? p.Tb : p.T) +
                                             ((int64_t)pos * WP_TILED + boot) * Q_BW + half * 64);
        for (int c = 0; c < 64; c += 8) {
            uint32_t r[8] = {0u, 0u, 0u, 0u, 0u, 0u, 0u, 0u};
            if (!empty_list) {
                tmem_ld_32x32b_x8(tcol + (uint32_t)c, r);
                tmem_wait_ld();
            }
            if (boot < p.n_boot) {
                dst[c / 4] = make_int4((int)r[0], (int)r[1], (int)r[2], (int)r[3]);
                dst[c / 4 + 1] = make_int4((int)r[4], (int)r[5], (int)r[6], (int)r[7]);
            }
        }
        tc_fence_before_sync();
        mbar_arrive(&sm.acc_empty);
    }
}

template <int Q_PGROUPS, bool HINT, int NS, bool BOUND>
__global__ void __launch_bounds__(q_threads(Q_PGROUPS), 1) contract_i8_kernel(const I8Params p) {
    static_assert(NS >= 2 && NS <= Q_NS, "ring depth");
    constexpr int Q_PRODUCER_WARPS = 4 * Q_PGROUPS;
    extern __shared__ __align__(1024) unsigned char smem_raw[];
    const uint32_t raw = smem_u32(smem_raw);
    const uint32_t stage0 = (raw + 1023u) & ~1023u;
    const uint32_t xbuf = stage0 + (uint32_t)NS * Q_STAGE_BYTES;
    I8Smem &sm = *reinterpret_cast<I8Smem *>(smem_raw + (stage0 - raw) + (size_t)NS * Q_STAGE_BYTES + Q_XBUF_BYTES);
    const int warp = threadIdx.x >> 5, lane = threadIdx.x & 31;
    if (threadIdx.x == 0) {
        for (int s = 0; s < NS; ++s) {
            mbar_init(&sm.full[s], 4 * 32);
            mbar_init(&sm.empty[s], 1);
        }
        mbar_init(&sm.acc_full, 1);
        mbar_init(&sm.acc_empty, Q_EPILOGUE_WARPS * 32);
        sm.abort = 0;
        mbar_fence_init();
    }
    if (warp == Q_PRODUCER_WARPS + Q_EPILOGUE_WARPS) tmem_alloc(&sm.tmem_base, Q_TMEM_COLS);
    tc_fence_before_sync();
    __syncthreads();
    tc_fence_after_sync();
    const uint32_t tmem = sm.tmem_base;
    const int n_items = (p.items ? *p.n_live : p.n_pos * p.n_pieces) << p.twin;

    if (warp < Q_PRODUCER_WARPS)
        run_producer<Q_PGROUPS, HINT, NS, BOUND>(p, sm, stage0, n_items, warp, lane);
    else if (warp < Q_PRODUCER_WARPS + Q_EPILOGUE_WARPS) {
        if (BOUND)
            run_bound_epilogue(p, sm, tmem, n_items, warp - Q_PRODUCER_WARPS, lane);
        else
            run_epilogue(p, sm, xbuf, tmem, n_items, warp - Q_PRODUCER_WARPS, lane);
    } else if (lane == 0)
        run_mma<NS, BOUND>(p, sm, stage0, tmem, n_items);

    tc_fence_before_sync();
    __syncthreads();
    tc_fence_after_sync();
    if (sm.abort && p.err && threadIdx.x == 0) atomicExch(p.err, 2);
    if (warp == Q_PRODUCER_WARPS + Q_EPILOGUE_WARPS) tmem_dealloc(tmem, Q_TMEM_COLS);
}

__global__ void __launch_bounds__(256) sentinel_range_kernel(const int32_t *__restrict__ lst_row, const int32_t *__restrict__ lst_cell,
                                                             const int32_t *__restrict__ lst_len, const int32_t *__restrict__ order,
                                                             int64_t ld_lst, const uint32_t *__restrict__ row_range,
                                                             const int8_t *__restrict__ W8, const int32_t *__restrict__ gene_set,
                                                             int64_t set_w8, int n_pos, int K, int n_boot,
                                                             uint32_t *__restrict__ SR, int32_t *__restrict__ flag) {
    const int pos = blockIdx.x * (blockDim.x >> 5) + (threadIdx.x >> 5);
    if (pos >= n_pos) return;
    const int lane = threadIdx.x & 31;
    const int64_t gene = order ? order[pos] : pos;
    if (gene_set) W8 += gene_set[gene] * set_w8;
    const int len = lst_len[gene];
    const int32_t *lr = lst_row + gene * ld_lst, *lc = lst_cell + gene * ld_lst;
    const uint32_t full = (uint32_t)(K - 1) << 16;
    uint32_t lo01 = 0u, lo23 = 0u, hi01 = 0xFFFFFFFFu, hi23 = 0xFFFFFFFFu;
    const uint32_t v01 = (4 * lane < n_boot ? 0xFFFFu : 0u) | (4 * lane + 1 < n_boot ? 0xFFFF0000u : 0u);
    const uint32_t v23 = (4 * lane + 2 < n_boot ? 0xFFFFu : 0u) | (4 * lane + 3 < n_boot ? 0xFFFF0000u : 0u);
    bool irregular = false;
    auto fetch = [&](int e0, uint32_t &rr, int32_t &cell) {
        const int e = e0 + lane;
        rr = full;
        cell = 0;
        if (e < len) {
            rr = __ldg(row_range + lr[e]);
            cell = lc[e] & ~LIST_HOT_BIT;
        }
    };
    uint32_t rr_n = full;
    int32_t cell_n = 0;
    if (len > 0) fetch(0, rr_n, cell_n);
    for (int e0 = 0; e0 < len; e0 += 32) {
        const uint32_t rr = rr_n;
        const int32_t cell = cell_n;
        if (e0 + 32 < len) fetch(e0 + 32, rr_n, cell_n);
        const uint32_t lmin2 = __vminu2(lo01 | ~v01, lo23 | ~v23), hmax2 = __vmaxu2(hi01 & v01, hi23 & v23);
        const uint32_t gmin = __reduce_min_sync(0xffffffffu, min(lmin2 & 0xFFFFu, lmin2 >> 16));
        const uint32_t gmax = __reduce_max_sync(0xffffffffu, max(hmax2 & 0xFFFFu, hmax2 >> 16));
        unsigned need = __ballot_sync(0xffffffffu, rr != full && (rr == Q_RANGE_IRREGULAR || (rr & 0xFFFFu) > gmin ||
                                                                  (rr >> 16) < gmax));
        while (need) {
            uint32_t r[4], w[4];
#pragma unroll
            for (int u = 0; u < 4; ++u) {
                r[u] = full;
                w[u] = 0u;
                if (need) {
                    const int src = __ffs(need) - 1;
                    need &= need - 1;
                    r[u] = __shfl_sync(0xffffffffu, rr, src);
                    const int32_t c = __shfl_sync(0xffffffffu, cell, src);
                    w[u] = __ldg(reinterpret_cast<const uint32_t *>(W8 + (int64_t)c * Q_WB + 4 * lane));
                }
            }
#pragma unroll
            for (int u = 0; u < 4; ++u) {
                if (r[u] == Q_RANGE_IRREGULAR) {
                    irregular = true;
                    continue;
                }
                const uint32_t m = __vcmpne4(w[u], 0u);
                const uint32_t m01 = __byte_perm(m, 0u, 0x1100), m23 = __byte_perm(m, 0u, 0x3322);
                const uint32_t klo2 = (r[u] & 0xFFFFu) * 0x10001u, khi2 = (r[u] >> 16) * 0x10001u;
                lo01 = __vmaxu2(lo01, klo2 & m01);
                lo23 = __vmaxu2(lo23, klo2 & m23);
                hi01 = __vminu2(hi01, khi2 | ~m01);
                hi23 = __vminu2(hi23, khi2 | ~m23);
            }
        }
    }
    uint32_t out[4];
    bool bad = irregular;
#pragma unroll
    for (int j = 0; j < 4; ++j) {
        const uint32_t lo = ((j < 2 ? lo01 : lo23) >> (16 * (j & 1))) & 0xFFFFu;
        uint32_t hi = ((j < 2 ? hi01 : hi23) >> (16 * (j & 1))) & 0xFFFFu;
        if (hi > (uint32_t)(K - 1)) hi = (uint32_t)(K - 1);
        if (4 * lane + j < n_boot && lo > hi) bad = true;
        out[j] = lo | (hi == (uint32_t)(K - 1) ? 0xFFFF0000u : hi << 16);
    }
    *reinterpret_cast<uint4 *>(SR + (int64_t)pos * Q_WB + 4 * lane) = make_uint4(out[0], out[1], out[2], out[3]);
    if (__any_sync(0xffffffffu, bad) && lane == 0) atomicOr(flag, 4);
}

constexpr int SP_GROUPS = 8, SP_ROWS = WP_TILED / SP_GROUPS;
static_assert(SP_GROUPS * SP_ROWS == WP_TILED && SP_ROWS * 32 == KP_TILED, "13 warps x 32 lanes = the 416 grid slots");
constexpr int SW_WARPS = 8;
template <bool SETS, bool LIVE>
__global__ void __launch_bounds__(SW_WARPS * 32, 2)
softmax_i8_warp_kernel(const long long *__restrict__ T, const double *__restrict__ Z, const uint32_t *__restrict__ SR, int K,
                       int n_boot_pass, double scale, double *__restrict__ part, int n_pos, const int32_t *__restrict__ order,
                       const int32_t *__restrict__ gene_set, int64_t set_z, const uint8_t *__restrict__ live) {
    constexpr int NJ = KP_TILED / 32;
    extern __shared__ double s_z[];
    const int group = blockIdx.x % SP_GROUPS, batch = blockIdx.x / SP_GROUPS, n_batch = gridDim.x / SP_GROUPS;
    const int warp = threadIdx.x >> 5, lane = threadIdx.x & 31;
    const int b0 = group * SP_ROWS;
    const int nb = min(SP_ROWS, n_boot_pass - b0);
    if (!SETS) {
        for (int i = threadIdx.x; i < SP_ROWS * KP_TILED; i += SW_WARPS * 32)
            s_z[i] = (Z && i / KP_TILED < nb) ? Z[(int64_t)b0 * KP_TILED + i] : 0.0;
        __syncthreads();
    }
    const double q = 1.0 / (double)(1ll << Q_FRAC);
    for (int pos = batch * SW_WARPS + warp; pos < n_pos; pos += n_batch * SW_WARPS) {
        double acc[NJ];
#pragma unroll
        for (int j = 0; j < NJ; ++j) acc[j] = 0.0;
        const long long *rows = T + ((int64_t)pos * WP_TILED + b0) * KP_TILED + lane;
        const uint32_t sr_l = (SR && lane < SP_ROWS) ? SR[(int64_t)pos * Q_WB + b0 + lane] : 0xFFFF0000u;
        const double *zg = s_z;
        if (SETS) zg = Z + gene_set[order ? order[pos] : pos] * set_z + (int64_t)b0 * KP_TILED;
        uint32_t lm = (1u << NJ) - 1u;
        if (LIVE) {
            const uint32_t pm = live[pos];
            lm = 0u;
#pragma unroll
            for (int j = 0; j < NJ; ++j) lm |= ((pm >> ((lane + 32 * j) / Q_PW)) & 1u) << j;
        }
        long long nxt[NJ];
        if (nb > 0) {
#pragma unroll
            for (int j = 0; j < NJ; ++j) nxt[j] = (lm >> j) & 1u ? __ldcs(rows + 32 * j) : 0ll;
        }
        for (int bi = 0; bi < nb; ++bi) {
            long long cur[NJ];
#pragma unroll
            for (int j = 0; j < NJ; ++j) cur[j] = nxt[j];
            if (bi + 1 < nb) {
                const long long *r2 = rows + (int64_t)(bi + 1) * KP_TILED;
#pragma unroll
                for (int j = 0; j < NJ; ++j) nxt[j] = (lm >> j) & 1u ? __ldcs(r2 + 32 * j) : 0ll;
            }
            const uint32_t sr = __shfl_sync(0xffffffffu, sr_l, bi);
            const int klo = (int)(sr & 0xFFFFu), span = min((int)(sr >> 16), K - 1) - klo;
            const double *zr = zg + bi * KP_TILED + lane;
            double v[NJ], m = -INFINITY;
#pragma unroll
            for (int j = 0; j < NJ; ++j) {
                const int k = lane + 32 * j;
                const double t = fma((double)cur[j], q, zr[32 * j]);
                v[j] = (unsigned)(k - klo) <= (unsigned)span && span >= 0 && ((lm >> j) & 1u) ? t : -INFINITY;
                m = v[j] > m ? v[j] : m;
            }
#pragma unroll
            for (int o = 16; o > 0; o >>= 1) {
                const double mo = __shfl_xor_sync(0xffffffffu, m, o);
                m = mo > m ? mo : m;
            }
            double sum = 0.0;
            uint32_t amask = 0u;
#pragma unroll
            for (int j = 0; j < NJ; ++j) {
                const double d = v[j] - m;
                v[j] = 0.0;
                if (__any_sync(0xffffffffu, d > -746.0)) {
                    v[j] = d > -INFINITY ? exp_nonpos(d) : 0.0;
                    amask |= 1u << j;
                }
                sum += v[j];
            }
#pragma unroll
            for (int o = 16; o > 0; o >>= 1) sum += __shfl_xor_sync(0xffffffffu, sum, o);
            const double inv = 1.0 / (sum * scale);
#pragma unroll
            for (int j = 0; j < NJ; ++j)
                if (amask & (1u << j)) acc[j] = __dadd_rn(acc[j], __dmul_rn(v[j], inv));
        }
        double *dst = part + ((int64_t)group * n_pos + pos) * KP_TILED + lane;
#pragma unroll
        for (int j = 0; j < NJ; ++j) dst[32 * j] = acc[j];
    }
}

__global__ void softmax_i8_reduce_kernel(const double *__restrict__ part, const int32_t *__restrict__ order, int K, int n_pos,
                                         double *__restrict__ jp, int64_t ld_jp, int accumulate) {
    const int64_t idx = (int64_t)blockIdx.x * blockDim.x + threadIdx.x;
    if (idx >= (int64_t)n_pos * KP_TILED) return;
    const int pos = (int)(idx / KP_TILED), k = (int)(idx - (int64_t)pos * KP_TILED);
    if (k >= K) return;
    double r = 0.0;
#pragma unroll
    for (int g = 0; g < SP_GROUPS; ++g) r += part[((int64_t)g * n_pos + pos) * KP_TILED + k];
    const int64_t gene = order ? order[pos] : pos;
    double *out = jp + gene * ld_jp + k;
    *out = accumulate ? *out + r : r;
}

__global__ void finalize_t_kernel(long long *__restrict__ T, const uint32_t *__restrict__ SR, double sentinel, int64_t n) {
    const int64_t idx = (int64_t)blockIdx.x * blockDim.x + threadIdx.x;
    if (idx >= n) return;
    const int k = (int)(idx % KP_TILED);
    const int64_t row = idx / KP_TILED;
    const int b = (int)(row % WP_TILED);
    const int64_t pos = row / WP_TILED;
    const uint32_t sr = SR ? SR[pos * Q_WB + b] : 0xFFFF0000u;
    double t = (double)T[idx] * (1.0 / (double)(1ll << Q_FRAC));
    if (k < (int)(sr & 0xFFFFu) || k > (int)(sr >> 16)) t = sentinel;
    reinterpret_cast<double *>(T)[idx] = t;
}


__global__ void z_bounds_kernel(const double *__restrict__ Z, int64_t n_rows, int K, double *__restrict__ zb) {
    const int64_t idx = (int64_t)blockIdx.x * blockDim.x + threadIdx.x;
    if (idx >= n_rows * Q_BSLOTS) return;
    const int64_t row = idx / Q_BSLOTS;
    const int s = (int)(idx - row * Q_BSLOTS);
    const double *z = Z + row * KP_TILED;
    double v = -INFINITY;
    if (s < Q_UB_N) {
        for (int k = s * Q_UB_PTS; k < (s + 1) * Q_UB_PTS && k < K; ++k) v = fmax(v, Z ? z[k] : 0.0);
    } else if (s < Q_UB_N + Q_LB_N) {
        const int k = Q_LB_STEP * (s - Q_UB_N) + Q_LB_OFF;
        if (k < K) v = Z ? z[k] : 0.0;
    }
    zb[idx] = v;
}

struct PruneSideDev {
    const uint32_t *sr;
    const int32_t *S;
    const double *zb;
    int n_boot;
};
__global__ void __launch_bounds__(256) prune_decide_kernel(PruneSideDev s0, PruneSideDev s1, int sides, const int32_t *__restrict__ order,
                                                           const int32_t *__restrict__ gene_set, int64_t set_zb, int n_pos, int K,
                                                           int n_pieces, uint8_t *__restrict__ live, double *__restrict__ lb_out,
                                                           double *__restrict__ ub_out) {
    const int pos = blockIdx.x * (blockDim.x >> 5) + (threadIdx.x >> 5);
    if (pos >= n_pos) return;
    const int lane = threadIdx.x & 31;
    const int64_t zoff = gene_set ? gene_set[order ? order[pos] : pos] * set_zb : 0;
    const uint32_t all = (1u << n_pieces) - 1u;
    uint32_t dead = all;
    for (int side = 0; side < sides; ++side) {
        const PruneSideDev s = side ? s1 : s0;
        for (int b = lane; b < s.n_boot; b += 32) {
            const uint32_t sr = s.sr ? s.sr[(int64_t)pos * Q_WB + b] : 0xFFFF0000u;
            const int klo = (int)(sr & 0xFFFFu), khi = min((int)(sr >> 16), K - 1);
            const int32_t *S = s.S + ((int64_t)pos * WP_TILED + b) * Q_BW;
            const double *z = s.zb + zoff + (int64_t)b * Q_BSLOTS;
            double lb = -INFINITY;
            for (int c = 0; c < Q_LB_N; ++c) {
                const int k = Q_LB_STEP * c + Q_LB_OFF;
                if (k >= klo && k <= khi)
                    lb = fmax(lb, z[Q_UB_N + c] + ((double)S[Q_UB_N + c] + 256.0 * S[Q_BSLOTS + Q_UB_N + c]) * (1.0 / 32.0));
            }
            double ub[4] = {-INFINITY, -INFINITY, -INFINITY, -INFINITY};
            for (int u = 0; u < Q_UB_N; ++u) {
                const int lo = max(u * Q_UB_PTS, klo), hi = min(u * Q_UB_PTS + Q_UB_PTS - 1, khi);
                if (lo > hi) continue;
                const double v = z[u] + ((double)S[u] + 256.0 * S[Q_BSLOTS + u]) * (1.0 / 32.0);
#pragma unroll
                for (int pc = 0; pc < 4; ++pc)
                    if (max(lo, pc * Q_PW) <= min(hi, pc * Q_PW + Q_PW - 1)) ub[pc] = fmax(ub[pc], v);
            }
            if (lb_out && side == 0) {
                lb_out[(int64_t)pos * WP_TILED + b] = lb;
                for (int pc = 0; pc < 4; ++pc) ub_out[((int64_t)pos * WP_TILED + b) * 4 + pc] = ub[pc];
            }
            const double thr = lb - 747.0;
            uint32_t d = 0u;
#pragma unroll
            for (int pc = 0; pc < 4; ++pc) d |= ub[pc] < thr ? 1u << pc : 0u;
            dead &= d;
        }
    }
    dead = __reduce_and_sync(0xffffffffu, dead);
    if (lane == 0) live[pos] = (uint8_t)(~dead & all);
}

constexpr int PC_THREADS = 1024;
__global__ void __launch_bounds__(PC_THREADS) prune_compact_kernel(const uint8_t *__restrict__ live, int n_pos, int n_pieces,
                                                                   int piece_major, const int32_t *__restrict__ order,
                                                                   const int32_t *__restrict__ lst_len, int32_t *__restrict__ items,
                                                                   int32_t *__restrict__ n_live, unsigned long long *stats) {
    __shared__ int wsum[PC_THREADS / 32];
    unsigned long long work = 0, live_work = 0;
    const int warp = threadIdx.x >> 5, lane = threadIdx.x & 31;
    const int n = n_pos * n_pieces;
    int base = 0;
    for (int i0 = 0; i0 < n; i0 += 4 * PC_THREADS) {
        uint32_t f = 0u;
        int c = 0;
#pragma unroll
        for (int e = 0; e < 4; ++e) {
            const int i = i0 + 4 * threadIdx.x + e;
            if (i < n) {
                const int piece = piece_major ? i / n_pos : i % n_pieces;
                const int pos = piece_major ? i - piece * n_pos : i / n_pieces;
                const unsigned long long len = stats ? (unsigned long long)max(lst_len[order ? order[pos] : pos], 0) : 0ull;
                work += len;
                if ((live[pos] >> piece) & 1u) {
                    f |= 1u << e;
                    ++c;
                    live_work += len;
                }
            }
        }
        int x = c;
#pragma unroll
        for (int o = 1; o < 32; o <<= 1) {
            const int y = __shfl_up_sync(0xffffffffu, x, o);
            if (lane >= o) x += y;
        }
        if (lane == 31) wsum[warp] = x;
        __syncthreads();
        if (warp == 0) {
            int w = wsum[lane];
#pragma unroll
            for (int o = 1; o < 32; o <<= 1) {
                const int y = __shfl_up_sync(0xffffffffu, w, o);
                if (lane >= o) w += y;
            }
            wsum[lane] = w;
        }
        __syncthreads();
        int off = base + (warp ? wsum[warp - 1] : 0) + x - c;
#pragma unroll
        for (int e = 0; e < 4; ++e)
            if ((f >> e) & 1u) items[off++] = i0 + 4 * threadIdx.x + e;
        base += wsum[PC_THREADS / 32 - 1];
        __syncthreads();
    }
    if (threadIdx.x == 0) {
        *n_live = base;
        if (stats) {
            atomicAdd(stats, (unsigned long long)n);
            atomicAdd(stats + 1, (unsigned long long)base);
        }
    }
    if (stats) {
        work = __reduce_add_sync(0xffffffffu, (unsigned)work) + 0ull;
        live_work = __reduce_add_sync(0xffffffffu, (unsigned)live_work) + 0ull;
        if (lane == 0) {
            atomicAdd(stats + 2, work);
            atomicAdd(stats + 3, live_work);
        }
    }
}

__global__ void exp_probe_kernel(double *out) {
    const int i = threadIdx.x;
    if (i < 3) out[i] = exp_nonpos(-745.0 - i);
}

__global__ void __launch_bounds__(256) quantize_rows_kernel(const double *__restrict__ table, int ld_table, int K, int64_t n_rows,
                                                            int8_t *__restrict__ qtable, int64_t ldq,
                                                            uint32_t *__restrict__ row_range, int8_t *__restrict__ qbound) {
    const int64_t row = (int64_t)blockIdx.x * (blockDim.x >> 5) + (threadIdx.x >> 5);
    if (row >= n_rows) return;
    const int lane = threadIdx.x & 31;
    const double *src = table + row * ld_table;
    int8_t *dst = qtable + row * ldq;
    for (int64_t j = lane; j < ldq / 4; j += 32) reinterpret_cast<uint32_t *>(dst)[j] = 0u;
    __syncwarp();
    int n_ok = 0, kmin = 0x7fffffff, kmax = -1;
    for (int k = lane; k < K; k += 32) {
        const double v = src[k];
        if (!(v > -1.0e290)) continue;
        ++n_ok;
        kmin = min(kmin, k);
        kmax = max(kmax, k);
        long long x = __double2ll_rn(fmin(fmax(v, -1000.0), 1000.0) * (double)(1ll << Q_FRAC));
        const int pc = k / Q_PW, i = k - pc * Q_PW;
#pragma unroll
        for (int pl = 0; pl < Q_NV; ++pl) {
            const int d = (int)(int8_t)(x & 0xFF);
            dst[pc * Q_PIECE + pl * Q_PW + i] = (int8_t)d;
            x = (x - d) >> 8;
        }
    }
#pragma unroll
    for (int o = 16; o > 0; o >>= 1) {
        n_ok += __shfl_xor_sync(0xffffffffu, n_ok, o);
        kmin = min(kmin, __shfl_xor_sync(0xffffffffu, kmin, o));
        kmax = max(kmax, __shfl_xor_sync(0xffffffffu, kmax, o));
    }
    uint32_t rr;
    if (n_ok == 0)
        rr = Q_RANGE_IRREGULAR;
    else if (kmax - kmin + 1 != n_ok)
        rr = Q_RANGE_IRREGULAR;
    else
        rr = (uint32_t)kmin | ((uint32_t)kmax << 16);
    if (lane == 0) row_range[row] = rr;
    if (qbound) {
        __syncwarp();
        q_bound_row(dst, K, rr, qbound + row * Q_BW, lane, 32);
    }
}

__global__ void w_to_i8_kernel(const double *__restrict__ W, int64_t n_rows_total, int8_t *__restrict__ W8,
                               int32_t *__restrict__ flag) {
    const int64_t idx = (int64_t)blockIdx.x * blockDim.x + threadIdx.x;
    if (idx >= n_rows_total * Q_WB) return;
    const int64_t row = idx / Q_WB;
    const int col = (int)(idx - row * Q_WB);
    int v = 0;
    if (col < WP_TILED) {
        const double w = W[row * WS_TILED + col];
        if (w > 127.0) {
            atomicOr(flag, 1);
            v = 127;
        } else {
            v = (int)w;
        }
    }
    W8[idx] = (int8_t)v;
}

}

cudaError_t launch_quantize_rows(const double *table, int ld_table, int K, int64_t n_rows, int8_t *qtable,
                                 uint32_t *row_range, int8_t *qbound, cudaStream_t st) {
    if (n_rows <= 0) return cudaSuccess;
    if (K > ld_table || K > Q_MAX_K) return cudaErrorInvalidValue;
    quantize_rows_kernel<<<(unsigned)((n_rows + 7) / 8), 256, 0, st>>>(table, ld_table, K, n_rows, qtable, q_row_bytes(K),
                                                                        row_range, qbound);
    return cudaGetLastError();
}

cudaError_t launch_w_to_i8(const double *W, int n_w_rows, int n_boot, int8_t *W8, int32_t *flag, cudaStream_t st) {
    const int passes = (n_boot + WP_TILED - 1) / WP_TILED;
    const int64_t rows = (int64_t)(passes > 0 ? passes : 1) * n_w_rows;
    const int64_t n = rows * Q_WB;
    w_to_i8_kernel<<<(unsigned)((n + 255) / 256), 256, 0, st>>>(W, rows, W8, flag);
    return cudaGetLastError();
}

bool contract_i8_supported(int K, int ld_table, int ld_lst, int n_draws) {
    return K >= 1 && K <= Q_MAX_K && ld_table == KP_TILED && (ld_lst % Q_ES) == 0 && n_draws <= 65000;
}

size_t contract_i8_range_words(int n_genes) { return (size_t)(n_genes > 0 ? n_genes : 1) * Q_WB; }

static int side_boots(const ContractI8Args &a, const I8Side &s) {
    return (a.n_boot - s.pass * WP_TILED) < WP_TILED ? (a.n_boot - s.pass * WP_TILED) : WP_TILED;
}

static I8Params make_params(const ContractI8Args &a, int g0, int n_pos, const I8Side *s, int n_sides) {
    I8Params p;
    p.qtable = a.qtable;
    p.ldq = a.ldq;
    p.lst_row = a.lists.row;
    p.lst_cell = a.lists.cell;
    p.lst_len = a.lists.len;
    p.order = a.lists.order ? a.lists.order + g0 : nullptr;
    p.ld_lst = a.lists.ld;
    p.W8 = s[0].W8;
    p.gene_set = a.gene_set;
    p.set_w8 = a.set_w8;
    p.T = reinterpret_cast<long long *>(s[0].T);
    p.n_boot = side_boots(a, s[0]);
    p.n_pos = n_pos;
    p.n_pieces = q_pieces(a.K);
    p.err = a.err;
    p.dbg = a.dbg;
    p.W8b = n_sides > 1 ? s[1].W8 : nullptr;
    p.Tb = n_sides > 1 ? reinterpret_cast<long long *>(s[1].T) : nullptr;
    p.twin = n_sides > 1 ? 1 : 0;
    p.piece_major = a.item_order == 1;
    p.cold_evict_first = a.cold_evict_first;
    p.items = a.items;
    p.n_live = a.items ? a.n_live : nullptr;
    return p;
}

cudaError_t launch_sentinel_ranges(const ContractI8Args &a, int g0, int n_pos, const I8Side &s, cudaStream_t st) {
    if (n_pos <= 0 || !a.row_range) return cudaSuccess;
    if (!s.SR) return cudaErrorInvalidValue;
    const I8Params p = make_params(a, g0, n_pos, &s, 1);
    sentinel_range_kernel<<<(unsigned)((n_pos + 7) / 8), 256, 0, st>>>(p.lst_row, p.lst_cell, p.lst_len, p.order, p.ld_lst,
                                                                       a.row_range, p.W8, a.gene_set, a.set_w8, n_pos, a.K,
                                                                       p.n_boot, s.SR, a.err);
    return cudaGetLastError();
}

cudaError_t launch_contract_i8_pass(const ContractI8Args &a, int g0, int n_pos, const I8Side *s, int n_sides, int n_sm,
                                    cudaStream_t st) {
    if (n_pos <= 0) return cudaSuccess;
    constexpr int PG = 1;
    const I8Params p = make_params(a, g0, n_pos, s, n_sides);
    const int n_items = (n_pos * p.n_pieces) << p.twin;
    int grid = n_sm < n_items ? n_sm : n_items;
    if (p.twin) grid &= ~1;
    auto launch = [&](auto kernel, int ns) -> cudaError_t {
        const size_t smem = q_smem_bytes(ns);
        cudaError_t e = cudaFuncSetAttribute(kernel, cudaFuncAttributeMaxDynamicSharedMemorySize, (int)smem);
        if (e != cudaSuccess) return e;
        kernel<<<grid, q_threads(PG), smem, st>>>(p);
        return cudaGetLastError();
    };
    if (a.hot_rank >= 0) return launch(contract_i8_kernel<PG, true, Q_NS, false>, Q_NS);
    if (a.ring_stages == 7) return launch(contract_i8_kernel<PG, false, 7, false>, 7);
    if (a.ring_stages == 8) return launch(contract_i8_kernel<PG, false, 8, false>, 8);
    return launch(contract_i8_kernel<PG, false, Q_NS, false>, Q_NS);
}

size_t prune_zb_doubles(int n_sets, int n_boot) {
    const int passes = (n_boot + WP_TILED - 1) / WP_TILED;
    return (size_t)(n_sets > 0 ? n_sets : 1) * (passes > 0 ? passes : 1) * WP_TILED * Q_BSLOTS;
}

cudaError_t launch_z_bounds(const ContractI8Args &a, const double *Z, int n_sets, double *zb, cudaStream_t st) {
    const int64_t rows = (int64_t)prune_zb_doubles(n_sets, a.n_boot) / Q_BSLOTS;
    z_bounds_kernel<<<(unsigned)((rows * Q_BSLOTS + 255) / 256), 256, 0, st>>>(Z, rows, a.K, zb);
    return cudaGetLastError();
}

size_t prune_bound_ints(int n_pos) { return (size_t)(n_pos > 0 ? n_pos : 1) * WP_TILED * Q_BW; }

cudaError_t launch_bound_pass(const ContractI8Args &a, int g0, int n_pos, const I8Side *s, int n_sides, int n_sm,
                              cudaStream_t st) {
    if (n_pos <= 0) return cudaSuccess;
    if (!a.qbound) return cudaErrorInvalidValue;
    constexpr int PG = 1;
    I8Params p = make_params(a, g0, n_pos, s, n_sides);
    p.qtable = a.qbound;
    p.ldq = Q_BW;
    p.n_pieces = 1;
    p.piece_major = 0;
    p.items = nullptr;
    p.n_live = nullptr;
    p.T = reinterpret_cast<long long *>(s[0].S);
    p.Tb = n_sides > 1 ? reinterpret_cast<long long *>(s[1].S) : nullptr;
    const int n_items = n_pos << p.twin;
    int grid = n_sm < n_items ? n_sm : n_items;
    if (p.twin) grid &= ~1;
    auto kernel = contract_i8_kernel<PG, false, Q_NS, true>;
    const size_t smem = q_smem_bytes(Q_NS);
    cudaError_t e = cudaFuncSetAttribute(kernel, cudaFuncAttributeMaxDynamicSharedMemorySize, (int)smem);
    if (e != cudaSuccess) return e;
    kernel<<<grid, q_threads(PG), smem, st>>>(p);
    return cudaGetLastError();
}

cudaError_t launch_prune_items(const ContractI8Args &a, int g0, int n_pos, const I8Side *s, int n_sides, uint8_t *live,
                               int32_t *items, int32_t *n_live, unsigned long long *stats, cudaStream_t st,
                               double *lb_out, double *ub_out) {
    if (n_pos <= 0) return cudaSuccess;
    const int32_t *order = a.lists.order ? a.lists.order + g0 : nullptr;
    auto dev = [&](const I8Side &x) {
        return PruneSideDev{a.row_range ? x.SR : nullptr, x.S, x.zb + (size_t)x.pass * WP_TILED * Q_BSLOTS, side_boots(a, x)};
    };
    const int64_t set_zb = (int64_t)prune_zb_doubles(1, a.n_boot);
    prune_decide_kernel<<<(unsigned)((n_pos + 7) / 8), 256, 0, st>>>(dev(s[0]), dev(s[n_sides - 1]), n_sides, order,
                                                                     a.gene_set, set_zb, n_pos, a.K, q_pieces(a.K), live,
                                                                     lb_out, ub_out);
    cudaError_t e = cudaGetLastError();
    if (e != cudaSuccess) return e;
    prune_compact_kernel<<<1, PC_THREADS, 0, st>>>(live, n_pos, q_pieces(a.K), a.item_order == 1, order, a.lists.len, items,
                                                   n_live, stats);
    return cudaGetLastError();
}

cudaError_t launch_exp_probe(double *out_host, cudaStream_t st) {
    double *d = nullptr;
    cudaError_t e = cudaMallocAsync(&d, 3 * sizeof(double), st);
    if (e != cudaSuccess) return e;
    exp_probe_kernel<<<1, 32, 0, st>>>(d);
    e = cudaGetLastError();
    if (e == cudaSuccess) e = cudaMemcpyAsync(out_host, d, 3 * sizeof(double), cudaMemcpyDeviceToHost, st);
    const cudaError_t f = cudaFreeAsync(d, st);
    return e != cudaSuccess ? e : f;
}

size_t softmax_i8_scratch_doubles(int n_pos) { return (size_t)SP_GROUPS * (n_pos > 0 ? n_pos : 1) * KP_TILED; }

cudaError_t launch_softmax_i8(const ContractI8Args &a, int g0, int n_pos, const I8Side &s, double *part_scratch, int n_sm,
                              cudaStream_t st, const uint8_t *live) {
    if (n_pos <= 0) return cudaSuccess;
    if (a.row_range && !s.SR) return cudaErrorInvalidValue;
    const bool sets = a.gene_set && s.Z;
    const size_t smem = sets ? 0 : sizeof(double) * SP_ROWS * KP_TILED;
    auto kernel = sets ? (live ? softmax_i8_warp_kernel<true, true> : softmax_i8_warp_kernel<true, false>)
                       : (live ? softmax_i8_warp_kernel<false, true> : softmax_i8_warp_kernel<false, false>);
    cudaError_t e = cudaFuncSetAttribute(kernel, cudaFuncAttributeMaxDynamicSharedMemorySize, (int)smem);
    if (e != cudaSuccess) return e;
    int wb = n_sm * 2 / SP_GROUPS;
    if (wb * SW_WARPS > n_pos) wb = (n_pos + SW_WARPS - 1) / SW_WARPS;
    if (wb < 1) wb = 1;
    kernel<<<wb * SP_GROUPS, SW_WARPS * 32, smem, st>>>(reinterpret_cast<const long long *>(s.T), s.Z,
                                                        a.row_range ? s.SR : nullptr, a.K, side_boots(a, s), a.scale,
                                                        part_scratch, n_pos, a.lists.order ? a.lists.order + g0 : nullptr,
                                                        a.gene_set, a.set_z, live);
    e = cudaGetLastError();
    if (e != cudaSuccess) return e;
    const int64_t n = (int64_t)n_pos * KP_TILED;
    softmax_i8_reduce_kernel<<<(unsigned)((n + 255) / 256), 256, 0, st>>>(part_scratch, a.lists.order ? a.lists.order + g0 : nullptr,
                                                                          a.K, n_pos, s.jp, a.ld_jp, s.pass > 0);
    return cudaGetLastError();
}

cudaError_t launch_finalize_t(const ContractI8Args &a, int n_pos, const I8Side &s, cudaStream_t st) {
    if (n_pos <= 0) return cudaSuccess;
    const int64_t n = (int64_t)n_pos * WP_TILED * KP_TILED;
    finalize_t_kernel<<<(unsigned)((n + 255) / 256), 256, 0, st>>>(reinterpret_cast<long long *>(s.T),
                                                                   a.row_range ? s.SR : nullptr, a.sentinel, n);
    return cudaGetLastError();
}

}
```

Baseline: 440,300.

## Fuse bound pass and prune decision into one dedicated tcgen05 bound kernel

Replaces the bound-mode instance of the contraction kernel, which wrote int32 bound sums to global memory and was followed by a separate decide kernel, with a dedicated bound kernel. Its epilogue reads the accumulators from tensor memory and computes the lower and upper bounds and live bits directly. It uses a deeper ring sized for the bound tile, multiple accumulator buffers, and both sides staged per stage, and it sets live flags with atomicOr after a memset. This removes the S scratch round trip and one launch per chunk, at the cost of a more complex warp-specialized kernel with new barrier logic.

```diff
diff --git a/scde_b200/csrc/api.cu b/scde_b200/csrc/api.cu
--- a/scde_b200/csrc/api.cu
+++ b/scde_b200/csrc/api.cu
@@ -380,7 +380,7 @@
     DBuf<int32_t> lst_row, lst_cell, lst_len, order;
     DBuf<unsigned long long> total;
     DBuf<double> zb[2];
-    DBuf<int32_t> S[2], items, n_live;
+    DBuf<int32_t> items, n_live;
     DBuf<uint8_t> live;
 };
 
@@ -441,12 +441,11 @@
     for (int i = 0; i < n_sides; ++i) {
         SCDE_CUDA(scr.T[i].ensure(contract_tiled_scratch_doubles(t.n_genes)));
         SCDE_CUDA(scr.SR[i].ensure(contract_i8_range_words(mp)));
-        if (prune) SCDE_CUDA(scr.S[i].ensure(prune_bound_ints(mp)));
     }
     SCDE_CUDA(scr.spart.ensure(softmax_i8_scratch_doubles(mp)));
     if (prune) {
         for (int j = 0; j < n_joints; ++j) SCDE_CUDA(scr.zb[j].ensure(prune_zb_doubles(sets.n, n_boot)));
-        SCDE_CUDA(scr.live.ensure((size_t)mp));
+        SCDE_CUDA(scr.live.ensure(prune_live_bytes(mp)));
         SCDE_CUDA(scr.items.ensure((size_t)mp * q_pieces(t.K)));
         SCDE_CUDA(scr.n_live.ensure(1));
         q.qbound = t.qb.p;
@@ -455,7 +454,7 @@
     }
     auto side = [&](int j, int ps, int i) {
         return I8Side{scr.W8[j].p + (size_t)ps * n_w_rows * Q_WB, scr.Z[j].p + (size_t)ps * WP_TILED * KP_TILED, scr.T[i].p,
-                      scr.SR[i].p, scr.S[i].p, scr.zb[j].p, joints[j].jp_dev, ps};
+                      scr.SR[i].p, scr.zb[j].p, joints[j].jp_dev, ps};
     };
     struct Launch {
         I8Side s[2];
@@ -485,9 +484,9 @@
             if (tm) tm->end(SCDE_B200_T_OTHER, e0, st, l.n);
             if (prune) {
                 e0 = tm ? tm->begin(st) : -1;
-                SCDE_CUDA(launch_bound_pass(q, g0, n_pos, l.s, l.n, ctx->n_sm, st));
-                SCDE_CUDA(launch_prune_items(q, g0, n_pos, l.s, l.n, scr.live.p, scr.items.p, scr.n_live.p, prune_stats, st));
-                if (tm) tm->end(SCDE_B200_T_BOUND, e0, st, 3);
+                SCDE_CUDA(launch_prune_items(q, g0, n_pos, l.s, l.n, ctx->n_sm, scr.live.p, scr.items.p, scr.n_live.p,
+                                             prune_stats, st));
+                if (tm) tm->end(SCDE_B200_T_BOUND, e0, st, 2);
             }
             e0 = tm ? tm->begin(st) : -1;
             SCDE_CUDA(launch_contract_i8_pass(q, g0, n_pos, l.s, l.n, ctx->n_sm, st));
@@ -1839,28 +1838,26 @@
     q.hot_rank = -1;
     q.cold_evict_first = 0;
     q.ring_stages = ctx->opt.ring_stages;
-    I8Side side{d_w.p, nullptr, d_t.p, d_sr.p, nullptr, nullptr, nullptr, 0};
+    I8Side side{d_w.p, nullptr, d_t.p, d_sr.p, nullptr, nullptr, 0};
     SCDE_CUDA(launch_sentinel_ranges(q, 0, n_genes, side, st));
     DBuf<int8_t> d_qb;
     DBuf<double> d_z, d_zb, d_lb, d_ub;
-    DBuf<int32_t> d_s, d_items, d_nlive;
+    DBuf<int32_t> d_items, d_nlive;
     DBuf<uint8_t> d_live;
     if (qbound) {
         TRY(upload(d_qb, qbound, (size_t)n_rows * Q_BW, st));
         if (z) TRY(upload(d_z, z, (size_t)WP_TILED * KP_TILED, st));
         q.qbound = d_qb.p;
         SCDE_CUDA(d_zb.ensure(prune_zb_doubles(1, WP_TILED)));
-        SCDE_CUDA(d_s.ensure(prune_bound_ints(n_genes)));
         SCDE_CUDA(d_lb.ensure((size_t)n_genes * WP_TILED));
         SCDE_CUDA(d_ub.ensure((size_t)n_genes * WP_TILED * 4));
-        SCDE_CUDA(d_live.ensure((size_t)n_genes));
+        SCDE_CUDA(d_live.ensure(prune_live_bytes(n_genes)));
         SCDE_CUDA(d_items.ensure((size_t)n_genes * q_pieces(n_grid)));
         SCDE_CUDA(d_nlive.ensure(1));
-        side.S = d_s.p;
         side.zb = d_zb.p;
         SCDE_CUDA(launch_z_bounds(q, z ? d_z.p : nullptr, 1, d_zb.p, st));
-        SCDE_CUDA(launch_bound_pass(q, 0, n_genes, &side, 1, ctx->n_sm, st));
-        SCDE_CUDA(launch_prune_items(q, 0, n_genes, &side, 1, d_live.p, d_items.p, d_nlive.p, nullptr, st, d_lb.p, d_ub.p));
+        SCDE_CUDA(launch_prune_items(q, 0, n_genes, &side, 1, ctx->n_sm, d_live.p, d_items.p, d_nlive.p, nullptr, st, d_lb.p,
+                                     d_ub.p));
     }
     SCDE_CUDA(launch_contract_i8_pass(q, 0, n_genes, &side, 1, ctx->n_sm, st));
     SCDE_CUDA(launch_finalize_t(q, n_genes, side, st));
diff --git a/scde_b200/csrc/common.cuh b/scde_b200/csrc/common.cuh
--- a/scde_b200/csrc/common.cuh
+++ b/scde_b200/csrc/common.cuh
@@ -182,7 +182,6 @@
     const double *Z;
     double *T;
     uint32_t *SR;
-    int32_t *S;
     const double *zb;
     double *jp;
     int pass;
@@ -198,10 +197,8 @@
                               cudaStream_t st, const uint8_t *live = nullptr);
 size_t prune_zb_doubles(int n_sets, int n_boot);
 cudaError_t launch_z_bounds(const ContractI8Args &a, const double *Z, int n_sets, double *zb, cudaStream_t st);
-size_t prune_bound_ints(int n_pos);
-cudaError_t launch_bound_pass(const ContractI8Args &a, int g0, int n_pos, const I8Side *s, int n_sides, int n_sm,
-                              cudaStream_t st);
-cudaError_t launch_prune_items(const ContractI8Args &a, int g0, int n_pos, const I8Side *s, int n_sides, uint8_t *live,
+size_t prune_live_bytes(int n_pos);
+cudaError_t launch_prune_items(const ContractI8Args &a, int g0, int n_pos, const I8Side *s, int n_sides, int n_sm, uint8_t *live,
                                int32_t *items, int32_t *n_live, unsigned long long *stats, cudaStream_t st,
                                double *lb_out = nullptr, double *ub_out = nullptr);
 cudaError_t launch_exp_probe(double *out_host, cudaStream_t st);
diff --git a/scde_b200/csrc/contract_i8.cu b/scde_b200/csrc/contract_i8.cu
--- a/scde_b200/csrc/contract_i8.cu
+++ b/scde_b200/csrc/contract_i8.cu
@@ -56,7 +56,8 @@
     const int32_t *n_live;
 };
 
-__device__ __forceinline__ bool wait_or_abort(I8Smem &sm, uint64_t *bar, uint32_t parity) {
+template <class Smem>
+__device__ __forceinline__ bool wait_or_abort(Smem &sm, uint64_t *bar, uint32_t parity) {
     if (mbar_try_wait(bar, parity)) return true;
     const long long t0 = clock64();
     while (!mbar_try_wait(bar, parity)) {
@@ -104,7 +105,7 @@
                  "l"(policy)
                  : "memory");
 }
-template <int Q_PGROUPS, bool HINT, int NS, bool BOUND>
+template <int Q_PGROUPS, bool HINT, int NS>
 __device__ __forceinline__ void run_producer(const I8Params &p, I8Smem &sm, uint32_t stage0, int n_items, int warp, int lane) {
     uint64_t pol_hot = 0, pol_cold = 0;
     if (HINT) {
@@ -137,7 +138,7 @@
             len_n = p.lst_len[gene_n];
             if (p.gene_set) wset_n = p.gene_set[gene_n] * p.set_w8;
         }
-        const int8_t *qbase = p.qtable + (BOUND ? 0 : (int64_t)it.piece * Q_PIECE) + l7 * 16;
+        const int8_t *qbase = p.qtable + (int64_t)it.piece * Q_PIECE + l7 * 16;
         const int8_t *wbase = ((p.twin && (item & 1)) ? p.W8b : p.W8) + l7 * 16 + wset;
         const int32_t *lrow = p.lst_row + gene * p.ld_lst + kg * 8 + l3;
         const int32_t *lcell = p.lst_cell + gene * p.ld_lst + kg * 8 + l3;
@@ -175,12 +176,7 @@
                     const int8_t *w0 = wbase + (int64_t)(cel0 & ~LIST_HOT_BIT) * Q_WB;
                     const int8_t *w1 = wbase + (int64_t)(cel1 & ~LIST_HOT_BIT) * Q_WB;
                     if (fill > 0 && !wait_or_abort(sm, &sm.empty[slot], (fill - 1) & 1u)) return;
-                    if (BOUND) {
-                        cp_async16_at<0, 0>(sB0, src0);
-                        cp_async16_at<0, 0>(sB1, src1);
-                        cp_async16_at<0, 0>(sA + d0, w0);
-                        cp_async16_at<0, 0>(sA + d1, w1);
-                    } else if (HINT) {
+                    if (HINT) {
                         const uint64_t pol0 = (cel0 & LIST_HOT_BIT) ? pol_hot : pol_cold;
                         const uint64_t pol1 = (cel1 & LIST_HOT_BIT) ? pol_hot : pol_cold;
                         cp_async16_hint_at<0, 0>(sB0, src0, pol0);
@@ -228,9 +224,9 @@
     }
 }
 
-template <int NS, bool BOUND>
+template <int NS>
 __device__ __forceinline__ void run_mma(const I8Params &p, I8Smem &sm, uint32_t stage0, uint32_t tmem, int n_items) {
-    const uint32_t idesc = umma_idesc_s8_mn(128, BOUND ? Q_BW : 256);
+    const uint32_t idesc = umma_idesc_s8_mn(128, 256);
     int slot = 0;
     uint32_t fill = 0, n_done = 0;
     int item = blockIdx.x;
@@ -252,7 +248,7 @@
             const uint32_t sB = sA + Q_A_BYTES;
             const uint64_t da = umma_desc_sw128(sA, 4096u, 1024u);
             umma_s8(tmem, da, umma_desc_sw128(sB, 4096u, 1024u), idesc, s > 0);
-            if (!BOUND) umma_s8(tmem + 256u, da, umma_desc_sw128(sB + 2u * 4096u, 4096u, 1024u), idesc, s > 0);
+            umma_s8(tmem + 256u, da, umma_desc_sw128(sB + 2u * 4096u, 4096u, 1024u), idesc, s > 0);
             umma_commit(&sm.empty[slot]);
             if (++slot == NS) {
                 slot = 0;
@@ -331,38 +327,7 @@
     }
 }
 
-__device__ __forceinline__ void run_bound_epilogue(const I8Params &p, I8Smem &sm, uint32_t tmem, int n_items, int ewarp, int lane) {
-    const int qd = ewarp & 3, half = ewarp >> 2;
-    const uint32_t tcol = tmem + ((uint32_t)(qd * 32) << 16) + (uint32_t)(half * 64);
-    const int boot = qd * 32 + lane;
-    uint32_t n_done = 0;
-    for (int item = blockIdx.x; item < n_items; item += gridDim.x, ++n_done) {
-        const int pos = item >> p.twin;
-        const bool empty_list = p.lst_len[p.order ? p.order[pos] : pos] <= 0;
-        while (!mbar_try_wait(&sm.acc_full, n_done & 1u)) {
-            __nanosleep(200);
-            if (sm.abort) return;
-        }
-        tc_fence_after_sync();
-        int4 *dst = reinterpret_cast<int4 *>(reinterpret_cast<int32_t *>((p.twin && (item & 1)) ? p.Tb : p.T) +
-                                             ((int64_t)pos * WP_TILED + boot) * Q_BW + half * 64);
-        for (int c = 0; c < 64; c += 8) {
-            uint32_t r[8] = {0u, 0u, 0u, 0u, 0u, 0u, 0u, 0u};
-            if (!empty_list) {
-                tmem_ld_32x32b_x8(tcol + (uint32_t)c, r);
-                tmem_wait_ld();
-            }
-            if (boot < p.n_boot) {
-                dst[c / 4] = make_int4((int)r[0], (int)r[1], (int)r[2], (int)r[3]);
-                dst[c / 4 + 1] = make_int4((int)r[4], (int)r[5], (int)r[6], (int)r[7]);
-            }
-        }
-        tc_fence_before_sync();
-        mbar_arrive(&sm.acc_empty);
-    }
-}
-
-template <int Q_PGROUPS, bool HINT, int NS, bool BOUND>
+template <int Q_PGROUPS, bool HINT, int NS>
 __global__ void __launch_bounds__(q_threads(Q_PGROUPS), 1) contract_i8_kernel(const I8Params p) {
     static_assert(NS >= 2 && NS <= Q_NS, "ring depth");
     constexpr int Q_PRODUCER_WARPS = 4 * Q_PGROUPS;
@@ -390,14 +355,11 @@
     const int n_items = (p.items ? *p.n_live : p.n_pos * p.n_pieces) << p.twin;
 
     if (warp < Q_PRODUCER_WARPS)
-        run_producer<Q_PGROUPS, HINT, NS, BOUND>(p, sm, stage0, n_items, warp, lane);
-    else if (warp < Q_PRODUCER_WARPS + Q_EPILOGUE_WARPS) {
-        if (BOUND)
-            run_bound_epilogue(p, sm, tmem, n_items, warp - Q_PRODUCER_WARPS, lane);
-        else
-            run_epilogue(p, sm, xbuf, tmem, n_items, warp - Q_PRODUCER_WARPS, lane);
-    } else if (lane == 0)
-        run_mma<NS, BOUND>(p, sm, stage0, tmem, n_items);
+        run_producer<Q_PGROUPS, HINT, NS>(p, sm, stage0, n_items, warp, lane);
+    else if (warp < Q_PRODUCER_WARPS + Q_EPILOGUE_WARPS)
+        run_epilogue(p, sm, xbuf, tmem, n_items, warp - Q_PRODUCER_WARPS, lane);
+    else if (lane == 0)
+        run_mma<NS>(p, sm, stage0, tmem, n_items);
 
     tc_fence_before_sync();
     __syncthreads();
@@ -623,57 +585,315 @@
     zb[idx] = v;
 }
 
-struct PruneSideDev {
-    const uint32_t *sr;
-    const int32_t *S;
-    const double *zb;
-    int n_boot;
+constexpr int B_TILE = Q_ES * Q_WB;
+constexpr int B_RING = 192 * 1024;
+template <int SIDES>
+struct BoundGeom {
+    static constexpr int STAGE = (SIDES + 1) * B_TILE;
+    static constexpr int NS = B_RING / STAGE;
+    static constexpr int NACC = Q_TMEM_COLS / (SIDES * Q_BW);
 };
-__global__ void __launch_bounds__(256) prune_decide_kernel(PruneSideDev s0, PruneSideDev s1, int sides, const int32_t *__restrict__ order,
-                                                           const int32_t *__restrict__ gene_set, int64_t set_zb, int n_pos, int K,
-                                                           int n_pieces, uint8_t *__restrict__ live, double *__restrict__ lb_out,
-                                                           double *__restrict__ ub_out) {
-    const int pos = blockIdx.x * (blockDim.x >> 5) + (threadIdx.x >> 5);
-    if (pos >= n_pos) return;
-    const int lane = threadIdx.x & 31;
-    const int64_t zoff = gene_set ? gene_set[order ? order[pos] : pos] * set_zb : 0;
-    const uint32_t all = (1u << n_pieces) - 1u;
-    uint32_t dead = all;
-    for (int side = 0; side < sides; ++side) {
-        const PruneSideDev s = side ? s1 : s0;
-        for (int b = lane; b < s.n_boot; b += 32) {
-            const uint32_t sr = s.sr ? s.sr[(int64_t)pos * Q_WB + b] : 0xFFFF0000u;
-            const int klo = (int)(sr & 0xFFFFu), khi = min((int)(sr >> 16), K - 1);
-            const int32_t *S = s.S + ((int64_t)pos * WP_TILED + b) * Q_BW;
-            const double *z = s.zb + zoff + (int64_t)b * Q_BSLOTS;
-            double lb = -INFINITY;
-            for (int c = 0; c < Q_LB_N; ++c) {
-                const int k = Q_LB_STEP * c + Q_LB_OFF;
-                if (k >= klo && k <= khi)
-                    lb = fmax(lb, z[Q_UB_N + c] + ((double)S[Q_UB_N + c] + 256.0 * S[Q_BSLOTS + Q_UB_N + c]) * (1.0 / 32.0));
-            }
-            double ub[4] = {-INFINITY, -INFINITY, -INFINITY, -INFINITY};
-            for (int u = 0; u < Q_UB_N; ++u) {
-                const int lo = max(u * Q_UB_PTS, klo), hi = min(u * Q_UB_PTS + Q_UB_PTS - 1, khi);
-                if (lo > hi) continue;
-                const double v = z[u] + ((double)S[u] + 256.0 * S[Q_BSLOTS + u]) * (1.0 / 32.0);
-#pragma unroll
-                for (int pc = 0; pc < 4; ++pc)
-                    if (max(lo, pc * Q_PW) <= min(hi, pc * Q_PW + Q_PW - 1)) ub[pc] = fmax(ub[pc], v);
-            }
-            if (lb_out && side == 0) {
-                lb_out[(int64_t)pos * WP_TILED + b] = lb;
-                for (int pc = 0; pc < 4; ++pc) ub_out[((int64_t)pos * WP_TILED + b) * 4 + pc] = ub[pc];
-            }
-            const double thr = lb - 747.0;
-            uint32_t d = 0u;
-#pragma unroll
-            for (int pc = 0; pc < 4; ++pc) d |= ub[pc] < thr ? 1u << pc : 0u;
-            dead &= d;
-        }
-    }
-    dead = __reduce_and_sync(0xffffffffu, dead);
-    if (lane == 0) live[pos] = (uint8_t)(~dead & all);
+template <int SIDES>
+struct BoundSmem {
+    uint64_t full[BoundGeom<SIDES>::NS], empty[BoundGeom<SIDES>::NS];
+    uint64_t acc_full[BoundGeom<SIDES>::NACC], acc_empty[BoundGeom<SIDES>::NACC];
+    uint64_t lb_full, lb_empty;
+    double lb[SIDES][Q_WB];
+    uint32_t tmem_base;
+    volatile int abort;
+};
+template <int SIDES>
+constexpr size_t bound_smem_bytes() { return 1024  + (size_t)B_RING + sizeof(BoundSmem<SIDES>); }
+
+struct BoundParams {
+    const int8_t *qbound;
+    const int32_t *lst_row, *lst_cell, *lst_len, *order;
+    int64_t ld_lst;
+    const int32_t *gene_set;
+    int64_t set_w8, set_zb;
+    const int8_t *W8[2];
+    const uint32_t *SR[2];
+    const double *zb[2];
+    int n_boot[2];
+    int n_pos, K, n_pieces;
+    uint32_t *live;
+    double *lb_out, *ub_out;
+};
+
+template <int SIDES>
+__device__ __forceinline__ void bound_producer(const BoundParams &p, BoundSmem<SIDES> &sm, uint32_t stage0, int warp, int lane) {
+    using G = BoundGeom<SIDES>;
+    const int kg = warp, l7 = lane & 7, l3 = lane >> 3;
+    const uint32_t d0 = (uint32_t)kg * 1024u + (uint32_t)l3 * 128u + (uint32_t)((l7 ^ l3) << 4);
+    const uint32_t d1 = (uint32_t)kg * 1024u + (uint32_t)(l3 + 4) * 128u + (uint32_t)((l7 ^ (l3 + 4)) << 4);
+    int slot = 0;
+    uint32_t fill = 0;
+    int pos = blockIdx.x;
+    int64_t gene_n = 0, wset_n = 0;
+    int len_n = 0;
+    if (pos < p.n_pos) {
+        gene_n = p.order ? p.order[pos] : pos;
+        len_n = p.lst_len[gene_n];
+        if (p.gene_set) wset_n = p.gene_set[gene_n] * p.set_w8;
+    }
+    for (; pos < p.n_pos; pos += gridDim.x) {
+        const int64_t gene = gene_n, wset = wset_n;
+        const int nst = (len_n + Q_ES - 1) / Q_ES;
+        if (pos + (int)gridDim.x < p.n_pos) {
+            gene_n = p.order ? p.order[pos + gridDim.x] : pos + gridDim.x;
+            len_n = p.lst_len[gene_n];
+            if (p.gene_set) wset_n = p.gene_set[gene_n] * p.set_w8;
+        }
+        const int8_t *qbase = p.qbound + l7 * 16;
+        const int8_t *wb0 = p.W8[0] + wset + l7 * 16;
+        const int8_t *wb1 = p.W8[SIDES - 1] + wset + l7 * 16;
+        const int32_t *lrow = p.lst_row + gene * p.ld_lst + kg * 8 + l3;
+        const int32_t *lcell = p.lst_cell + gene * p.ld_lst + kg * 8 + l3;
+        int32_t r0a = 0, r1a = 0, c0a = 0, c1a = 0, r0b = 0, r1b = 0, c0b = 0, c1b = 0;
+        auto load_block = [&](int t, int32_t &r0, int32_t &r1, int32_t &c0, int32_t &c1) {
+            const int s = 8 * t + l7;
+            r0 = r1 = c0 = c1 = 0;
+            if (s < nst) {
+                r0 = __ldg(lrow + s * Q_ES);
+                r1 = __ldg(lrow + s * Q_ES + 4);
+                c0 = __ldg(lcell + s * Q_ES);
+                c1 = __ldg(lcell + s * Q_ES + 4);
+            }
+        };
+        load_block(0, r0a, r1a, c0a, c1a);
+        load_block(1, r0b, r1b, c0b, c1b);
+        for (int t = 0; 8 * t < nst; ++t) {
+#pragma unroll
+            for (int u = 0; u < 8; ++u) {
+                if (8 * t + u < nst) {
+                    const int from = (lane & 24) | u;
+                    const int32_t row0 = __shfl_sync(0xffffffffu, r0a, from), row1 = __shfl_sync(0xffffffffu, r1a, from);
+                    const int64_t cel0 = __shfl_sync(0xffffffffu, c0a, from) & ~LIST_HOT_BIT;
+                    const int64_t cel1 = __shfl_sync(0xffffffffu, c1a, from) & ~LIST_HOT_BIT;
+                    const uint32_t sA = stage0 + (uint32_t)slot * G::STAGE, sB = sA + SIDES * B_TILE;
+                    if (fill > 0 && !wait_or_abort(sm, &sm.empty[slot], (fill - 1) & 1u)) return;
+                    cp_async16_at<0, 0>(sB + d0, qbase + (int64_t)row0 * Q_BW);
+                    cp_async16_at<0, 0>(sB + d1, qbase + (int64_t)row1 * Q_BW);
+                    cp_async16_at<0, 0>(sA + d0, wb0 + cel0 * Q_WB);
+                    cp_async16_at<0, 0>(sA + d1, wb0 + cel1 * Q_WB);
+                    if (SIDES > 1) {
+                        cp_async16_at<B_TILE, 0>(sA + d0, wb1 + cel0 * Q_WB);
+                        cp_async16_at<B_TILE, 0>(sA + d1, wb1 + cel1 * Q_WB);
+                    }
+                    cp_async_mbar_arrive_noinc(&sm.full[slot]);
+                    if (++slot == G::NS) {
+                        slot = 0;
+                        ++fill;
+                    }
+                }
+            }
+            r0a = r0b;
+            r1a = r1b;
+            c0a = c0b;
+            c1a = c1b;
+            load_block(t + 2, r0b, r1b, c0b, c1b);
+        }
+    }
+}
+
+template <int SIDES>
+__device__ __forceinline__ void bound_mma(const BoundParams &p, BoundSmem<SIDES> &sm, uint32_t stage0, uint32_t tmem) {
+    using G = BoundGeom<SIDES>;
+    const uint32_t idesc = umma_idesc_s8_mn(128, Q_BW);
+    int slot = 0;
+    uint32_t fill = 0, n_done = 0;
+    int pos = blockIdx.x;
+    int len_n = pos < p.n_pos ? p.lst_len[p.order ? p.order[pos] : pos] : 0;
+    for (; pos < p.n_pos; pos += gridDim.x, ++n_done) {
+        const int nst = (len_n + Q_ES - 1) / Q_ES;
+        if (pos + (int)gridDim.x < p.n_pos) len_n = p.lst_len[p.order ? p.order[pos + gridDim.x] : pos + gridDim.x];
+        const int buf = (int)(n_done % G::NACC);
+        const uint32_t use = n_done / G::NACC;
+        if (use > 0) {
+            if (!wait_or_abort(sm, &sm.acc_empty[buf], (use - 1) & 1u)) return;
+            tc_fence_after_sync();
+        }
+        const uint32_t acc = tmem + (uint32_t)(buf * SIDES * Q_BW);
+        for (int s = 0; s < nst; ++s) {
+            if (!wait_or_abort(sm, &sm.full[slot], fill & 1u)) return;
+            fence_proxy_async_smem();
+            tc_fence_after_sync();
+            const uint32_t sA = stage0 + (uint32_t)slot * G::STAGE;
+            const uint64_t db = umma_desc_sw128(sA + SIDES * B_TILE, 4096u, 1024u);
+#pragma unroll
+            for (int side = 0; side < SIDES; ++side)
+                umma_s8(acc + (uint32_t)(side * Q_BW), umma_desc_sw128(sA + side * B_TILE, 4096u, 1024u), db, idesc, s > 0);
+            umma_commit(&sm.empty[slot]);
+            if (++slot == G::NS) {
+                slot = 0;
+                ++fill;
+            }
+        }
+        if (nst > 0)
+            umma_commit(&sm.acc_full[buf]);
+        else
+            mbar_arrive(&sm.acc_full[buf]);
+    }
+}
+
+template <int SIDES>
+__device__ __forceinline__ bool bound_wait(BoundSmem<SIDES> &sm, uint64_t *bar, uint32_t parity) {
+    while (!mbar_try_wait(bar, parity)) {
+        __nanosleep(100);
+        if (sm.abort) return false;
+    }
+    return true;
+}
+
+template <int SIDES>
+__device__ __forceinline__ void bound_epilogue(const BoundParams &p, BoundSmem<SIDES> &sm, uint32_t tmem, int ewarp, int lane) {
+    using G = BoundGeom<SIDES>;
+    const int qd = ewarp & 3, half = ewarp >> 2;
+    const int boot = qd * 32 + lane;
+    const uint32_t tq = tmem + ((uint32_t)(qd * 32) << 16);
+    const uint32_t all = (1u << p.n_pieces) - 1u;
+    uint32_t n_done = 0;
+    for (int pos = blockIdx.x; pos < p.n_pos; pos += gridDim.x, ++n_done) {
+        const int64_t gene = p.order ? p.order[pos] : pos;
+        const bool empty_list = p.lst_len[gene] <= 0;
+        const int64_t zoff = p.gene_set ? p.gene_set[gene] * p.set_zb : 0;
+        int klo[SIDES], khi[SIDES];
+        const double *zr[SIDES];
+#pragma unroll
+        for (int side = 0; side < SIDES; ++side) {
+            const uint32_t sr = p.SR[side] ? p.SR[side][(int64_t)pos * Q_WB + boot] : 0xFFFF0000u;
+            klo[side] = (int)(sr & 0xFFFFu);
+            khi[side] = min((int)(sr >> 16), p.K - 1);
+            zr[side] = p.zb[side] + zoff + (int64_t)(boot < p.n_boot[side] ? boot : 0) * Q_BSLOTS;
+        }
+        const int buf = (int)(n_done % G::NACC);
+        if (!bound_wait(sm, &sm.acc_full[buf], (n_done / G::NACC) & 1u)) return;
+        tc_fence_after_sync();
+        auto load8 = [&](int side, int j, uint32_t (&lo)[8], uint32_t (&hi)[8]) {
+#pragma unroll
+            for (int i = 0; i < 8; ++i) lo[i] = hi[i] = 0u;
+            if (!empty_list) {
+                const uint32_t col = tq + (uint32_t)(buf * SIDES * Q_BW + side * Q_BW + 8 * j);
+                tmem_ld_32x32b_x8(col, lo);
+                tmem_ld_32x32b_x8(col + Q_BSLOTS, hi);
+                tmem_wait_ld();
+            }
+        };
+        if (half) {
+            double lb[SIDES];
+#pragma unroll
+            for (int side = 0; side < SIDES; ++side) {
+                lb[side] = -INFINITY;
+#pragma unroll
+                for (int j = Q_UB_N / 8; j < (Q_UB_N + Q_LB_N + 7) / 8; ++j) {
+                    uint32_t lo[8], hi[8];
+                    load8(side, j, lo, hi);
+#pragma unroll
+                    for (int i = 0; i < 8; ++i) {
+                        const int slot = 8 * j + i;
+                        if (slot < Q_UB_N || slot >= Q_UB_N + Q_LB_N) continue;
+                        const int k = Q_LB_STEP * (slot - Q_UB_N) + Q_LB_OFF;
+                        if (k >= klo[side] && k <= khi[side])
+                            lb[side] = fmax(lb[side], zr[side][slot] + ((double)(int32_t)lo[i] + 256.0 * (int32_t)hi[i]) * (1.0 / 32.0));
+                    }
+                }
+            }
+            tc_fence_before_sync();
+            mbar_arrive(&sm.acc_empty[buf]);
+            if (n_done > 0 && !bound_wait(sm, &sm.lb_empty, (n_done - 1) & 1u)) return;
+#pragma unroll
+            for (int side = 0; side < SIDES; ++side) sm.lb[side][boot] = lb[side];
+            mbar_arrive(&sm.lb_full);
+        } else {
+            double ub[SIDES][4];
+#pragma unroll
+            for (int side = 0; side < SIDES; ++side) {
+#pragma unroll
+                for (int pc = 0; pc < 4; ++pc) ub[side][pc] = -INFINITY;
+#pragma unroll
+                for (int j = 0; j < (Q_UB_N + 7) / 8; ++j) {
+                    uint32_t lo[8], hi[8];
+                    load8(side, j, lo, hi);
+#pragma unroll
+                    for (int i = 0; i < 8; ++i) {
+                        const int u = 8 * j + i;
+                        if (u >= Q_UB_N) continue;
+                        const int bl = max(u * Q_UB_PTS, klo[side]), bh = min(u * Q_UB_PTS + Q_UB_PTS - 1, khi[side]);
+                        if (bl > bh) continue;
+                        const double v = zr[side][u] + ((double)(int32_t)lo[i] + 256.0 * (int32_t)hi[i]) * (1.0 / 32.0);
+#pragma unroll
+                        for (int pc = 0; pc < 4; ++pc)
+                            if (max(bl, pc * Q_PW) <= min(bh, pc * Q_PW + Q_PW - 1)) ub[side][pc] = fmax(ub[side][pc], v);
+                    }
+                }
+            }
+            tc_fence_before_sync();
+            mbar_arrive(&sm.acc_empty[buf]);
+            if (!bound_wait(sm, &sm.lb_full, n_done & 1u)) return;
+            double lb[SIDES];
+#pragma unroll
+            for (int side = 0; side < SIDES; ++side) lb[side] = sm.lb[side][boot];
+            mbar_arrive(&sm.lb_empty);
+            uint32_t dead = all;
+#pragma unroll
+            for (int side = 0; side < SIDES; ++side) {
+                if (boot >= p.n_boot[side]) continue;
+                if (side == 0 && p.lb_out) {
+                    p.lb_out[(int64_t)pos * WP_TILED + boot] = lb[0];
+                    for (int pc = 0; pc < 4; ++pc) p.ub_out[((int64_t)pos * WP_TILED + boot) * 4 + pc] = ub[0][pc];
+                }
+                const double thr = lb[side] - 747.0;
+                uint32_t d = 0u;
+#pragma unroll
+                for (int pc = 0; pc < 4; ++pc) d |= ub[side][pc] < thr ? 1u << pc : 0u;
+                dead &= d;
+            }
+            dead = __reduce_and_sync(0xffffffffu, dead);
+            const uint32_t lv = ~dead & all;
+            if (lane == 0 && lv) atomicOr(p.live + (pos >> 2), lv << (8 * (pos & 3)));
+        }
+    }
+}
+
+template <int SIDES>
+__global__ void __launch_bounds__(q_threads(1), 1) bound_i8_kernel(const BoundParams p, int32_t *err) {
+    using G = BoundGeom<SIDES>;
+    constexpr int PRODUCER_WARPS = 4;
+    extern __shared__ __align__(1024) unsigned char smem_raw[];
+    const uint32_t raw = smem_u32(smem_raw);
+    const uint32_t stage0 = (raw + 1023u) & ~1023u;
+    BoundSmem<SIDES> &sm = *reinterpret_cast<BoundSmem<SIDES> *>(smem_raw + (stage0 - raw) + B_RING);
+    const int warp = threadIdx.x >> 5, lane = threadIdx.x & 31;
+    if (threadIdx.x == 0) {
+        for (int s = 0; s < G::NS; ++s) {
+            mbar_init(&sm.full[s], 4 * 32);
+            mbar_init(&sm.empty[s], 1);
+        }
+        for (int b = 0; b < G::NACC; ++b) {
+            mbar_init(&sm.acc_full[b], 1);
+            mbar_init(&sm.acc_empty[b], Q_EPILOGUE_WARPS * 32);
+        }
+        mbar_init(&sm.lb_full, Q_EPILOGUE_WARPS / 2 * 32);
+        mbar_init(&sm.lb_empty, Q_EPILOGUE_WARPS / 2 * 32);
+        sm.abort = 0;
+        mbar_fence_init();
+    }
+    if (warp == PRODUCER_WARPS + Q_EPILOGUE_WARPS) tmem_alloc(&sm.tmem_base, Q_TMEM_COLS);
+    tc_fence_before_sync();
+    __syncthreads();
+    tc_fence_after_sync();
+    const uint32_t tmem = sm.tmem_base;
+    if (warp < PRODUCER_WARPS)
+        bound_producer<SIDES>(p, sm, stage0, warp, lane);
+    else if (warp < PRODUCER_WARPS + Q_EPILOGUE_WARPS)
+        bound_epilogue<SIDES>(p, sm, tmem, warp - PRODUCER_WARPS, lane);
+    else if (lane == 0)
+        bound_mma<SIDES>(p, sm, stage0, tmem);
+    tc_fence_before_sync();
+    __syncthreads();
+    tc_fence_after_sync();
+    if (sm.abort && err && threadIdx.x == 0) atomicExch(err, 2);
+    if (warp == PRODUCER_WARPS + Q_EPILOGUE_WARPS) tmem_dealloc(tmem, Q_TMEM_COLS);
 }
 
 constexpr int PC_THREADS = 1024;
@@ -898,10 +1118,10 @@
         kernel<<<grid, q_threads(PG), smem, st>>>(p);
         return cudaGetLastError();
     };
-    if (a.hot_rank >= 0) return launch(contract_i8_kernel<PG, true, Q_NS, false>, Q_NS);
-    if (a.ring_stages == 7) return launch(contract_i8_kernel<PG, false, 7, false>, 7);
-    if (a.ring_stages == 8) return launch(contract_i8_kernel<PG, false, 8, false>, 8);
-    return launch(contract_i8_kernel<PG, false, Q_NS, false>, Q_NS);
+    if (a.hot_rank >= 0) return launch(contract_i8_kernel<PG, true, Q_NS>, Q_NS);
+    if (a.ring_stages == 7) return launch(contract_i8_kernel<PG, false, 7>, 7);
+    if (a.ring_stages == 8) return launch(contract_i8_kernel<PG, false, 8>, 8);
+    return launch(contract_i8_kernel<PG, false, Q_NS>, Q_NS);
 }
 
 size_t prune_zb_doubles(int n_sets, int n_boot) {
@@ -915,51 +1135,50 @@
     return cudaGetLastError();
 }
 
-size_t prune_bound_ints(int n_pos) { return (size_t)(n_pos > 0 ? n_pos : 1) * WP_TILED * Q_BW; }
-
-cudaError_t launch_bound_pass(const ContractI8Args &a, int g0, int n_pos, const I8Side *s, int n_sides, int n_sm,
-                              cudaStream_t st) {
-    if (n_pos <= 0) return cudaSuccess;
-    if (!a.qbound) return cudaErrorInvalidValue;
-    constexpr int PG = 1;
-    I8Params p = make_params(a, g0, n_pos, s, n_sides);
-    p.qtable = a.qbound;
-    p.ldq = Q_BW;
-    p.n_pieces = 1;
-    p.piece_major = 0;
-    p.items = nullptr;
-    p.n_live = nullptr;
-    p.T = reinterpret_cast<long long *>(s[0].S);
-    p.Tb = n_sides > 1 ? reinterpret_cast<long long *>(s[1].S) : nullptr;
-    const int n_items = n_pos << p.twin;
-    int grid = n_sm < n_items ? n_sm : n_items;
-    if (p.twin) grid &= ~1;
-    auto kernel = contract_i8_kernel<PG, false, Q_NS, true>;
-    const size_t smem = q_smem_bytes(Q_NS);
-    cudaError_t e = cudaFuncSetAttribute(kernel, cudaFuncAttributeMaxDynamicSharedMemorySize, (int)smem);
-    if (e != cudaSuccess) return e;
-    kernel<<<grid, q_threads(PG), smem, st>>>(p);
-    return cudaGetLastError();
-}
-
-cudaError_t launch_prune_items(const ContractI8Args &a, int g0, int n_pos, const I8Side *s, int n_sides, uint8_t *live,
+cudaError_t launch_prune_items(const ContractI8Args &a, int g0, int n_pos, const I8Side *s, int n_sides, int n_sm, uint8_t *live,
                                int32_t *items, int32_t *n_live, unsigned long long *stats, cudaStream_t st,
                                double *lb_out, double *ub_out) {
     if (n_pos <= 0) return cudaSuccess;
-    const int32_t *order = a.lists.order ? a.lists.order + g0 : nullptr;
-    auto dev = [&](const I8Side &x) {
-        return PruneSideDev{a.row_range ? x.SR : nullptr, x.S, x.zb + (size_t)x.pass * WP_TILED * Q_BSLOTS, side_boots(a, x)};
+    if (!a.qbound || n_sides < 1 || n_sides > 2) return cudaErrorInvalidValue;
+    BoundParams p{};
+    p.qbound = a.qbound;
+    p.lst_row = a.lists.row;
+    p.lst_cell = a.lists.cell;
+    p.lst_len = a.lists.len;
+    p.order = a.lists.order ? a.lists.order + g0 : nullptr;
+    p.ld_lst = a.lists.ld;
+    p.gene_set = a.gene_set;
+    p.set_w8 = a.set_w8;
+    p.set_zb = (int64_t)prune_zb_doubles(1, a.n_boot);
+    for (int i = 0; i < n_sides; ++i) {
+        p.W8[i] = s[i].W8;
+        p.SR[i] = a.row_range ? s[i].SR : nullptr;
+        p.zb[i] = s[i].zb + (size_t)s[i].pass * WP_TILED * Q_BSLOTS;
+        p.n_boot[i] = side_boots(a, s[i]);
+    }
+    p.n_pos = n_pos;
+    p.K = a.K;
+    p.n_pieces = q_pieces(a.K);
+    p.live = reinterpret_cast<uint32_t *>(live);
+    p.lb_out = lb_out;
+    p.ub_out = ub_out;
+    cudaError_t e = cudaMemsetAsync(live, 0, prune_live_bytes(n_pos), st);
+    if (e != cudaSuccess) return e;
+    const int grid = n_sm < n_pos ? n_sm : n_pos;
+    auto launch = [&](auto kernel, size_t smem) -> cudaError_t {
+        cudaError_t e = cudaFuncSetAttribute(kernel, cudaFuncAttributeMaxDynamicSharedMemorySize, (int)smem);
+        if (e != cudaSuccess) return e;
+        kernel<<<grid, q_threads(1), smem, st>>>(p, a.err);
+        return cudaGetLastError();
     };
-    const int64_t set_zb = (int64_t)prune_zb_doubles(1, a.n_boot);
-    prune_decide_kernel<<<(unsigned)((n_pos + 7) / 8), 256, 0, st>>>(dev(s[0]), dev(s[n_sides - 1]), n_sides, order,
-                                                                     a.gene_set, set_zb, n_pos, a.K, q_pieces(a.K), live,
-                                                                     lb_out, ub_out);
-    cudaError_t e = cudaGetLastError();
+    e = n_sides > 1 ? launch(bound_i8_kernel<2>, bound_smem_bytes<2>()) : launch(bound_i8_kernel<1>, bound_smem_bytes<1>());
     if (e != cudaSuccess) return e;
-    prune_compact_kernel<<<1, PC_THREADS, 0, st>>>(live, n_pos, q_pieces(a.K), a.item_order == 1, order, a.lists.len, items,
+    prune_compact_kernel<<<1, PC_THREADS, 0, st>>>(live, n_pos, q_pieces(a.K), a.item_order == 1, p.order, a.lists.len, items,
                                                    n_live, stats);
     return cudaGetLastError();
 }
+
+size_t prune_live_bytes(int n_pos) { return (size_t)((n_pos > 0 ? n_pos : 1) + 3) & ~(size_t)3; }
 
 cudaError_t launch_exp_probe(double *out_host, cudaStream_t st) {
     double *d = nullptr;
```

New measurement: 469,500 (median of 6 runs). 1.07x the previous value.
